# MrOlm/inStrain

Hardware: AMD Instinct MI355X
Metric: Gbp profiled/s (higher is better)
Workload: dtype u32

## Files before the change

include/instrain_amd.h:

```cpp
#ifndef INSTRAIN_AMD_H
#define INSTRAIN_AMD_H

#include <stdint.h>

#ifdef __cplusplus
extern "C" {
#endif

#define ISX_OK 0
#define ISX_ERR_ARG (-1)
#define ISX_ERR_HIP (-2)
#define ISX_ERR_CAPACITY (-3)
#define ISX_ERR_MM_RANGE (-4)
#define ISX_ERR_IO (-5)
#define ISX_ERR_STATE (-6)

#define ISX_ABI_VERSION 5


typedef struct isx_ctx isx_ctx;
typedef struct isx_batch isx_batch;
typedef struct isx_bam isx_bam;
struct isx_bam_params_s;
struct isx_bam_info_s;
// ... 393 lines not shown
    int32_t lev_mask_bytes, lev_cov_bytes, lev_window, n_lev_windows, lev_min_cov, pad_lev;
    uint64_t rows_checksum;
} isx_pipe_result;

int isx_levels_expand(const isx_pipe_result *r, int32_t host_threads, uint32_t *gpos, uint32_t *mm_cov, float *clon, float *clon_rarefied);

int isx_pipe_create(isx_ctx *ctx, const isx_params *params, const isx_pipe_params *pp, isx_pipe **out);
void isx_pipe_destroy(isx_pipe *p);
int isx_pipe_submit(isx_pipe *p, int64_t n_pos, const uint8_t *ref, int32_t n_splits, const int64_t *split_bounds,
                    int64_t n_obs, const isx_obs *obs, const uint32_t *pair, int64_t *ticket);
int isx_pipe_submit_bam(isx_pipe *p, isx_bam *bam, const struct isx_bam_params_s *bp, const int32_t *refs, int32_t n_refs,
                        const uint8_t *ref, int32_t n_splits, const int64_t *split_bounds, struct isx_bam_info_s *info,
                        int64_t *ticket);
int isx_pipe_collect(isx_pipe *p, int64_t ticket, isx_pipe_result *out);
int isx_pipe_release(isx_pipe *p, int64_t ticket);
int isx_pipe_fetch_entries(isx_pipe *p, int64_t ticket, isx_entry *out);
int isx_pipe_fetch_entries_shrunk(isx_pipe *p, int64_t ticket, uint32_t *gpos, uint32_t *mm_cov, float *clon, float *clon_rarefied);


#define ISX_SEG_BASES 150
#define ISX_SEG_WORDS 15
#define ISX_SEG_SKIP_WORD 0x24924924u
#define ISX_DREC_WORDS 8
#define ISX_DREC_EXC 6
#define ISX_DREC_EXC_FULL 3
#define ISX_DREC_DUAL 0x80000000u
#define ISX_DREC_NO_EXC 0x3FFFFFFFu

typedef struct {
    int64_t n_seg;
    const uint32_t *gpos;
    const uint8_t *len;
    const uint8_t *mm;
    const uint32_t *pair;
    const uint32_t *bases;
} isx_segs;

int isx_batch_create_reads(isx_ctx *ctx, const isx_params *params, int64_t n_pos, const uint8_t *ref, int32_t n_splits,
                           const int64_t *split_bounds, const isx_segs *segs, isx_batch **out);
int isx_pipe_submit_reads(isx_pipe *p, int64_t n_pos, const uint8_t *ref, int32_t n_splits, const int64_t *split_bounds,
                          const isx_segs *segs, int64_t *ticket);

typedef struct isx_wire isx_wire;
int isx_pipe_stage_reads(isx_pipe *p, int64_t n_pos, const uint8_t *ref, int32_t n_splits, const int64_t *split_bounds,
                         const isx_segs *segs, isx_wire **out);
int isx_pipe_submit_wire(isx_pipe *p, const isx_wire *wire, int64_t *ticket);
int64_t isx_wire_bytes(const isx_wire *wire);
void isx_wire_free(isx_wire *wire);
int isx_wire_keep_reference(isx_pipe *p, isx_wire *wire);

#define ISX_PLANE_WORDS 8
typedef struct {
    int64_t n_seg;
    const uint32_t *gpos;
    const uint8_t *len;
    const uint32_t *pair;
    const uint64_t *planes;
    const uint8_t *mm;
} isx_read_planes;

typedef struct {
    const uint8_t *plane2;
    const uint8_t *nplane;
    uint64_t key;
} isx_ref_planes;

int isx_pack_ref_planes(const uint8_t *ref, int64_t n_pos, int32_t host_threads, uint8_t *plane2, uint8_t *nplane, int32_t *has_n);
int isx_planes_from_segs(const isx_segs *segs, int32_t host_threads, uint64_t *planes);
int isx_pack_read_planes(int64_t n_reads, const int64_t *ref_start, const int64_t *clip_lo, const int64_t *clip_hi,
                         const uint32_t *cigar, const int64_t *cigar_off, const char *seq, const uint8_t *qual, const int64_t *seq_off,
                         const uint32_t *pair, int32_t min_base_quality, int64_t cap_seg, uint32_t *seg_gpos,
                         uint8_t *seg_len, uint32_t *seg_pair, uint64_t *seg_planes, int64_t *n_seg);
int isx_pipe_submit_planes(isx_pipe *p, int64_t n_pos, const isx_ref_planes *ref, int32_t n_splits, const int64_t *split_bounds,
                           const isx_read_planes *reads, int64_t *ticket);
int isx_pipe_stage_planes(isx_pipe *p, int64_t n_pos, const isx_ref_planes *ref, int32_t n_splits, const int64_t *split_bounds,
                          const isx_read_planes *reads, isx_wire **out);
int isx_pipe_set_reference_budget(isx_pipe *p, int64_t mib);
int isx_host_register(const void *ptr, int64_t bytes);
int isx_host_unregister(const void *ptr);
int isx_encode_planes(const isx_read_planes *reads, const isx_ref_planes *ref, int64_t n_pos, int32_t host_threads, int32_t slack_groups,
                      int64_t cap_rec, int64_t ring_records, uint32_t *rec, uint32_t *gbase, int64_t *n_rec, int64_t *need_slack);
int isx_encode_planes_mm(const isx_read_planes *reads, const isx_ref_planes *ref, int64_t n_pos, int32_t n_mm_bins, int32_t host_threads, int32_t slack_groups,
                         int64_t cap_rec, int64_t ring_records, uint32_t *rec, uint32_t *gbase, int64_t *n_rec, int64_t *need_slack);

int isx_count_read_segs(int64_t n_reads, const uint32_t *cigar, const int64_t *cigar_off, const int64_t *ref_start,
                        const int64_t *clip_lo, const int64_t *clip_hi, int64_t *n_seg);
int isx_pack_reads(int64_t n_reads, const int64_t *ref_start, const int64_t *clip_lo, const int64_t *clip_hi,
                   const uint32_t *cigar, const int64_t *cigar_off, const char *seq, const uint8_t *qual, const int64_t *seq_off,
                   const uint8_t *mm, const uint32_t *pair, int32_t min_base_quality, int64_t cap_seg, uint32_t *seg_gpos,
                   uint8_t *seg_len, uint8_t *seg_mm, uint32_t *seg_pair, uint32_t *seg_bases, int64_t *n_seg);

int isx_encode_segs(const isx_segs *segs, int64_t n_pos, int32_t n_mm_bins, int32_t host_threads, int64_t cap_rec, uint32_t *rec,
                    uint32_t *gbase, uint32_t *pair_out, int64_t *n_rec);
int64_t isx_seg_records_needed(const uint32_t *gpos, int64_t n_seg, int32_t host_threads);
int isx_encode_segs_ring(const isx_segs *segs, int64_t n_pos, int32_t n_mm_bins, int32_t host_threads, int64_t cap_rec, int64_t ring_records,
                         uint32_t *rec, uint32_t *gbase, uint32_t *pair_out, int64_t *n_rec);

int isx_encode_delta(const isx_segs *segs, const uint8_t *ref, int64_t n_pos, int32_t n_mm_bins, int32_t host_threads, int32_t slack_groups,
                     int64_t cap_rec, int64_t ring_records, uint32_t *rec, uint32_t *gbase, uint32_t *pair_out, int64_t *n_rec, int64_t *need_slack);
int64_t isx_delta_records_needed(const uint32_t *gpos, int64_t n_seg, int32_t host_threads, int32_t slack_groups);

int isx_encode_obs(const isx_obs *obs, const uint32_t *pair, int64_t n_obs, int64_t n_pos, int32_t record_bytes,
                   int32_t host_threads, double slack, int64_t cap_rec, void *rec, uint32_t *gbase, uint32_t *pair_out,
                   int64_t *n_rec, int32_t *passes);
int isx_encode_obs_ring(const isx_obs *obs, const uint32_t *pair, int64_t n_obs, int64_t n_pos, int32_t record_bytes,
                        int32_t host_threads, double slack, int64_t cap_rec, int64_t ring_records, void *rec,
                        uint32_t *gbase, uint32_t *pair_out, int64_t *n_rec, int32_t *passes);

typedef struct {
    int64_t in_off;
    int32_t in_len;
    int32_t out_len;
    int64_t out_off;
} isx_bgzf_block;
int isx_bgzf_index(const uint8_t *image, int64_t n_bytes, int64_t cap_blocks, isx_bgzf_block *blocks, int64_t *n_blocks, int64_t *out_bytes);
int isx_bgzf_inflate_device(isx_ctx *ctx, const uint8_t *image, int64_t n_bytes, const isx_bgzf_block *blocks, int64_t n_blocks,
                            uint8_t *out, int64_t out_bytes, float *kernel_ms);
int isx_bgzf_inflate_host(const uint8_t *image, int64_t n_bytes, const isx_bgzf_block *blocks, int64_t n_blocks, uint8_t *out, int64_t out_bytes);
int isx_bgzf_inflate_fast(const uint8_t *image, int64_t n_bytes, const isx_bgzf_block *blocks, int64_t n_blocks, uint8_t *out, int64_t out_bytes);

typedef struct isx_bam_params_s {
    double min_read_ani;
    int32_t min_mapq;
    double max_insert_relative;
    int32_t min_insert;
    int32_t min_base_quality;
    int32_t skip_mm;
    int32_t window_length;
    int32_t pairing_filter;
} isx_bam_params;

typedef struct isx_bam_info_s {
    int32_t n_refs;
    int32_t n_splits;
    int64_t n_reads;
    int64_t n_pos;
    int64_t n_obs;
    int64_t n_pairs;
    int64_t unfiltered_pairs, filtered_pairs;
    int64_t filtered_bases;
    double median_insert;
    int32_t max_mm;
    int32_t pad;
    int64_t unfiltered_reads, unfiltered_singletons, filtered_singletons;
    int64_t n_segs;
} isx_bam_info;

int isx_bam_open(const char *path, isx_bam **out);
void isx_bam_close(isx_bam *bam);
void isx_bam_close_wait(isx_bam *bam);
int isx_bam_set_threads(isx_bam *bam, int32_t threads);
int isx_bam_ref(const isx_bam *bam, int32_t i, const char **name, int64_t *length, int64_t *flat_offset);
int isx_bam_set_priority_reads(isx_bam *bam, int64_t n, const char *names, const int64_t *offs);
int isx_bam_scan(isx_bam *bam, isx_bam_info *info );
int isx_bam_scan_part(isx_bam *bam, int32_t part, int32_t n_parts, isx_bam_info *info );
int isx_bam_set_wanted_refs(isx_bam *bam, const int32_t *refs, int32_t n);
int isx_bam_insert_sizes(isx_bam *bam, int64_t *out, int64_t cap, int64_t *n);
int isx_bam_filter(isx_bam *bam, const isx_bam_params *p, double median_insert , isx_bam_info *info);
int isx_bam_pair_keys(isx_bam *bam, uint64_t *h1, uint64_t *h2, int32_t *tid, int64_t *info4, int64_t cap, int64_t *n);
int isx_bam_set_cross_names(isx_bam *bam, int64_t n, const int64_t *entry, const int64_t *occurrences, const int64_t *info4);
int isx_bam_filter_insert_sizes(isx_bam *bam, int64_t *out, int64_t cap, int64_t *n);
int isx_bam_set_r2m(isx_bam *bam, int32_t ref, int64_t n, const char *names, const int64_t *offs, const int32_t *mm );
int isx_bam_set_mm_cap(isx_bam *bam, int32_t cap);
int isx_bam_mm_levels(const isx_bam *bam, int32_t *levels, int32_t cap, int32_t *n);
int isx_bam_set_mm_levels(isx_bam *bam, const int32_t *levels, int32_t n);
int isx_bam_batch_pair_names(const isx_bam *bam, int64_t *n, int64_t *name_bytes, char *names, int64_t *offs);
// ... 18 lines not shown
```

instrain_amd/_lib.py:

```python
import ctypes as C
import os

import numpy as np

_HERE = os.path.dirname(os.path.abspath(__file__))
LIB_PATH = os.path.join(_HERE, "libinstrain_amd.so")
if os.environ.get("ISX_LIB"):
    LIB_PATH = os.path.abspath(os.environ["ISX_LIB"])

BGZF_BLOCK_DT = np.dtype([("in_off", np.int64), ("in_len", np.int32), ("out_len", np.int32), ("out_off", np.int64)])
OBS_DT = np.dtype([("gpos", "<u4"), ("mm", "<u2"), ("base", "u1"), ("flags", "u1")])
ENTRY_DT = np.dtype([("gpos", "<u4"), ("mm", "<u2"), ("flags", "<u2"), ("cnt", "<u4", (4,)), ("clon", "<f4"),
                     ("clon_rarefied", "<f4")])
SNV_DT = np.dtype([("gpos", "<u4"), ("mm", "<u2"), ("con_base", "u1"), ("var_base", "u1"),
                   ("allele_count", "u1"), ("cls", "u1"), ("cryptic", "u1"), ("ref_base", "u1"),
                   ("cnt", "<u4", (4,))])
LD_DT = np.dtype([("gpos_a", "<u4"), ("gpos_b", "<u4"), ("mm", "<u2"), ("allele_A", "u1"), ("allele_a", "u1"),
                  ("allele_B", "u1"), ("allele_b", "u1"), ("pad", "<u2"), ("total", "<u4"), ("countAB", "<u4"),
                  ("countAb", "<u4"), ("countaB", "<u4"), ("countab", "<u4"), ("pad2", "<u4"),
                  ("r2", "<f8"), ("d_prime", "<f8"), ("r2_normalized", "<f8"), ("d_prime_normalized", "<f8")])
AO_DT = np.dtype([("pair", "<u4"), ("gpos", "<u4"), ("order", "<u4"), ("mm", "<u2"), ("base", "u1"), ("pad", "u1")])
assert AO_DT.itemsize == 16
assert OBS_DT.itemsize == 8 and ENTRY_DT.itemsize == 32 and SNV_DT.itemsize == 28 and LD_DT.itemsize == 72

# ... 73 lines not shown


class BamParams(C.Structure):
    _fields_ = [("min_read_ani", C.c_double), ("min_mapq", C.c_int32), ("max_insert_relative", C.c_double),
                ("min_insert", C.c_int32), ("min_base_quality", C.c_int32), ("skip_mm", C.c_int32),
                ("window_length", C.c_int32), ("pairing_filter", C.c_int32)]


PAIRING_FILTERS = {"paired_only": 0, "non_discordant": 1, "all_reads": 2}


class BamInfo(C.Structure):
    _fields_ = [("n_refs", C.c_int32), ("n_splits", C.c_int32), ("n_reads", C.c_int64), ("n_pos", C.c_int64),
                ("n_obs", C.c_int64), ("n_pairs", C.c_int64), ("unfiltered_pairs", C.c_int64),
                ("filtered_pairs", C.c_int64), ("filtered_bases", C.c_int64), ("median_insert", C.c_double),
                ("max_mm", C.c_int32), ("pad", C.c_int32), ("unfiltered_reads", C.c_int64),
                ("unfiltered_singletons", C.c_int64), ("filtered_singletons", C.c_int64), ("n_segs", C.c_int64)]


SCAFFOLD_LEVEL_DT = np.dtype([("nonzero", "<i8"), ("sum_cov", "<u8"), ("sumsq_cov", "<u8"), ("median_cov", "<f8"),
                              ("counted", "<i8"), ("sum_clon", "<f8"), ("median_clon", "<f8"),
                              ("counted_rarefied", "<i8"), ("sum_clon_rarefied", "<f8"),
                              ("median_clon_rarefied", "<f8"), ("mm", "<i4"), ("present", "<i4")])
assert SCAFFOLD_LEVEL_DT.itemsize == 88
GENOME_LEVEL_DT = np.dtype([("n", "<i8"), ("sum_cov", "<u8"), ("sumsq_cov", "<u8"), ("median_cov", "<f8"), ("mm", "<i4"), ("pad", "<i4")])
assert GENOME_LEVEL_DT.itemsize == 40
GENOME_COV_DT = np.dtype([("n", "<i8"), ("sum_cov", "<u8"), ("sumsq_cov", "<u8"), ("max_cov", "<u4"), ("pad", "<u4")])
SNV_LEVEL_DT = np.dtype([(n, "<u4") for n in ("divergent", "sns", "snv", "con", "pop")])
LD_LEVEL_DT = np.dtype([("n", "<i8"), ("n_r2", "<i8"), ("n_dprime", "<i8"), ("sum_distance", "<i8"), ("sum_r2", "<f8"), ("sum_dprime", "<f8")])
assert GENOME_COV_DT.itemsize == 32 and SNV_LEVEL_DT.itemsize == 20 and LD_LEVEL_DT.itemsize == 48


COMPARE_LEVEL_DT = np.dtype([("both", "<i8"), ("either", "<i8"), ("mm", "<i4"), ("present_a", "<i4"),
                             ("present_b", "<i4"), ("pad", "<i4"), ("consensus_snps", "<i8"), ("population_snps", "<i8")])
assert COMPARE_LEVEL_DT.itemsize == 48
COMPARE_SNP_DT = np.dtype([("gpos", "<u4"), ("mm", "<u2"), ("consensus_snp", "u1"), ("population_snp", "u1"),
                           ("has_a", "u1"), ("has_b", "u1"), ("con_a", "u1"), ("ref_a", "u1"), ("var_a", "u1"),
                           ("con_b", "u1"), ("ref_b", "u1"), ("var_b", "u1"), ("cnt_a", "<u4", (4,)), ("cnt_b", "<u4", (4,))])
assert COMPARE_SNP_DT.itemsize == 48
IREP_WINDOW, IREP_SLIDE = 5000, 100
IREP_GENOME_DT = np.dtype([("L", "<i8"), ("n_blocks", "<i8"), ("n_windows", "<i8"), ("first_block", "<i8"), ("first_window", "<i8"),
                           ("first_scaffold", "<i4"), ("num_contigs", "<i4")])
IREP_ROW_DT = np.dtype([("L", "<i8"), ("n_windows", "<i8"), ("n_kept", "<i8"), ("sum_cov", "<u8"), ("avg_cov", "<f8"), ("fragMbp", "<f8"),
                        ("kept_windows", "<f8"), ("r2", "<f8"), ("raw_irep", "<f8"), ("gc_irep", "<f8"), ("irep", "<f8"),
                        ("num_contigs", "<i4"), ("flags", "<u4")])
assert IREP_GENOME_DT.itemsize == 48 and IREP_ROW_DT.itemsize == 96
IREP_FAIL_KEPT, IREP_FAIL_COV, IREP_FAIL_R2, IREP_FAIL_FRAG, IREP_EMPTY, IREP_NO_FIT = 1, 2, 4, 8, 16, 32
CMPSET_TILE_DT = np.dtype([("word0", "<i8"), ("n_words", "<i4"), ("scaffold", "<i4")])
CMPSET_MAX_LEVELS = 128
POOL_SITE_DT = np.dtype([("gpos", "<u4"), ("n_detect", "<u4"), ("cnt", "<u8", (4,)), ("n_detect_5x", "<u4"), ("cls_count", "<u2", (5,)),
                         ("ref_base", "u1"), ("con_base", "u1"), ("var_base", "u1"), ("n_con_bases", "u1"), ("con_bases", "u1"),
                         ("pad", "u1", (5,))])
assert POOL_SITE_DT.itemsize == 64
POOL_META_HAS, POOL_META_OWN = 1, 2


GENE_DT = np.dtype([("start", "<i8"), ("end", "<i8"), ("seq_off", "<i8"), ("strand", "<i4"), ("pad", "<i4")])
GENE_COV_DT = np.dtype([("sum_cov", "<u8"), ("nonzero", "<u4"), ("counted", "<u4"), ("sum_clon", "<f8")])
GENE_SNV_COUNT_DT = np.dtype([(n, "<u4") for n in ("divergent", "sns", "sns_n", "sns_s", "snv", "snv_n", "snv_s")])
GENE_MUTATION_DT = np.dtype([("gene", "<i4"), ("k", "<i4"), ("type", "u1"), ("aa_old", "u1"), ("aa_new", "u1"), ("n_genes", "u1"),
                             ("pad", "<u4")])
assert GENE_DT.itemsize == 32 and GENE_COV_DT.itemsize == 24 and GENE_SNV_COUNT_DT.itemsize == 28 and GENE_MUTATION_DT.itemsize == 16
GENE_LEVEL_PRESENT, GENE_COV_ANY, GENE_CLON_ANY = 1, 2, 4


ERR_CAPACITY = -3


class IsxError(RuntimeError):
    def __init__(self, code, msg):
        super().__init__("libinstrain_amd error %d: %s" % (code, msg))
        self.code = code


SYMBOLS = ["isx_last_error", "isx_abi_version", "isx_ctx_create", "isx_ctx_destroy", "isx_ctx_reserve_cus", "isx_set_null_model",
           "isx_batch_create", "isx_batch_create_reads", "isx_batch_destroy", "isx_batch_run", "isx_batch_launch", "isx_batch_wait", "isx_batch_sizes", "isx_batch_timings", "isx_batch_link_chain",
           "isx_batch_fetch_entries", "isx_batch_fetch_dense", "isx_batch_fetch_snv", "isx_batch_fetch_ld", "isx_batch_fetch_allele_obs",
           "isx_batch_summarize", "isx_batch_summarize_genomes", "isx_batch_genome_coverage", "isx_snv_level_counts", "isx_ld_level_sums", "isx_compare_coverage", "isx_compare_scaffolds", "isx_compare_fetch_snps",
           "isx_cmpset_layout", "isx_cmpset_tiles", "isx_cmpset_level_map", "isx_cmpset_create", "isx_cmpset_destroy", "isx_cmpset_add", "isx_cmpset_axis", "isx_cmpset_compare", "isx_cmpset_pair_snps", "isx_cmpset_fetch_snps",
           "isx_cmpset_pool_enable", "isx_cmpset_pool_sites", "isx_cmpset_pool_fetch_sites", "isx_cmpset_pool_add", "isx_cmpset_pool_summary", "isx_cmpset_pool_fetch_sample",
           "isx_irep_layout", "isx_irep_create", "isx_irep_destroy", "isx_irep_sizes", "isx_irep_add", "isx_irep_blocks_fetch", "isx_irep_blocks_add", "isx_irep_finish",
           "isx_genes_create", "isx_genes_destroy", "isx_genes_sites", "isx_batch_profile_genes", "isx_genes_profile_snvs",
           "isx_pipe_create", "isx_pipe_destroy", "isx_pipe_submit", "isx_pipe_submit_reads", "isx_pipe_stage_reads", "isx_pipe_submit_wire", "isx_wire_bytes", "isx_wire_free", "isx_wire_keep_reference", "isx_pipe_submit_bam", "isx_encode_segs", "isx_encode_segs_ring", "isx_seg_records_needed", "isx_encode_delta", "isx_delta_records_needed", "isx_count_read_segs", "isx_pack_reads", "isx_pipe_collect", "isx_pipe_release", "isx_pipe_fetch_entries", "isx_pipe_fetch_entries_shrunk", "isx_levels_expand", "isx_encode_obs", "isx_encode_obs_ring",
           "isx_pack_ref_planes", "isx_planes_from_segs", "isx_pack_read_planes", "isx_pipe_submit_planes", "isx_pipe_stage_planes", "isx_encode_planes", "isx_encode_planes_mm", "isx_pipe_set_reference_budget", "isx_host_register", "isx_host_unregister",
           "isx_bgzf_index", "isx_bgzf_inflate_device", "isx_bgzf_inflate_host", "isx_bgzf_inflate_fast",
           "isx_bam_open", "isx_bam_close", "isx_bam_close_wait", "isx_bam_set_threads", "isx_bam_ref", "isx_bam_set_priority_reads", "isx_bam_scan", "isx_bam_scan_part",
           "isx_bam_insert_sizes", "isx_bam_set_wanted_refs", "isx_bam_pair_keys", "isx_bam_set_cross_names", "isx_bam_filter_insert_sizes", "isx_bam_filter", "isx_bam_set_r2m", "isx_bam_r2m", "isx_bam_drop_names", "isx_bam_batch_pair_names", "isx_bam_set_mm_cap", "isx_bam_mm_levels", "isx_bam_set_mm_levels", "isx_bam_ref_counts",
           "isx_bam_expand_refs", "isx_bam_segment_refs", "isx_bam_copy_segs", "isx_bam_copy_read_planes", "isx_bam_expand_region", "isx_bam_expand", "isx_bam_copy", "isx_bam_view"]

_lib = None


def load():
    global _lib
    if _lib is not None:
        return _lib
    if not os.path.exists(LIB_PATH):
        raise IsxError(-2, "%s not built: run `python -c 'import __graft_entry__ as g; g.build()'` "
                           "(hipcc --offload-arch=gfx950)" % LIB_PATH)
    lib = C.CDLL(LIB_PATH)
    vp, i32, i64 = C.c_void_p, C.c_int32, C.c_int64
    lib.isx_last_error.restype = C.c_char_p
    lib.isx_abi_version.restype = C.c_int
    if lib.isx_abi_version() != ABI_VERSION:
        raise IsxError(-6, "%s has ABI version %d, this package binds version %d: rebuild it (python -c 'import __graft_entry__ as g; g.build()')"
                       % (LIB_PATH, lib.isx_abi_version(), ABI_VERSION))
    lib.isx_ctx_create.argtypes = [C.c_int, C.POINTER(vp)]
    lib.isx_ctx_destroy.argtypes = [vp]
    lib.isx_ctx_reserve_cus.argtypes = [vp, C.c_int]
    lib.isx_bgzf_index.argtypes = [vp, i64, i64, vp, C.POINTER(i64), C.POINTER(i64)]
    lib.isx_bgzf_inflate_device.argtypes = [vp, vp, i64, vp, i64, vp, i64, C.POINTER(C.c_float)]
    lib.isx_bgzf_inflate_host.argtypes = [vp, i64, vp, i64, vp, i64]
    lib.isx_bgzf_inflate_fast.argtypes = [vp, i64, vp, i64, vp, i64]
    lib.isx_ctx_destroy.restype = None
    lib.isx_set_null_model.argtypes = [vp, vp, i64, i32]
    lib.isx_batch_create.argtypes = [vp, C.POINTER(Params), i64, vp, i32, vp, i64, vp, vp, C.POINTER(vp)]
    lib.isx_batch_create_reads.argtypes = [vp, C.POINTER(Params), i64, vp, i32, vp, C.POINTER(Segs), C.POINTER(vp)]
    lib.isx_pipe_submit_reads.argtypes = [vp, i64, vp, i32, vp, C.POINTER(Segs), C.POINTER(i64)]
    lib.isx_pipe_stage_reads.argtypes = [vp, i64, vp, i32, vp, C.POINTER(Segs), C.POINTER(vp)]
    lib.isx_pipe_submit_wire.argtypes = [vp, vp, C.POINTER(i64)]
    lib.isx_wire_bytes.argtypes = [vp]
    lib.isx_wire_bytes.restype = i64
    lib.isx_wire_free.argtypes = [vp]
    lib.isx_wire_keep_reference.argtypes = [vp, vp]
    lib.isx_wire_free.restype = None
    lib.isx_encode_segs.argtypes = [C.POINTER(Segs), i64, i32, i32, i64, vp, vp, vp, C.POINTER(i64)]
    lib.isx_encode_segs_ring.argtypes = [C.POINTER(Segs), i64, i32, i32, i64, i64, vp, vp, vp, C.POINTER(i64)]
    lib.isx_encode_delta.argtypes = [C.POINTER(Segs), vp, i64, i32, i32, i32, i64, i64, vp, vp, vp, C.POINTER(i64), C.POINTER(i64)]
    lib.isx_delta_records_needed.argtypes = [vp, i64, i32, i32]
    lib.isx_delta_records_needed.restype = i64
    lib.isx_seg_records_needed.argtypes = [vp, i64, i32]
    lib.isx_seg_records_needed.restype = i64
    lib.isx_count_read_segs.argtypes = [i64, vp, vp, vp, vp, vp, C.POINTER(i64)]
    lib.isx_pack_reads.argtypes = [i64, vp, vp, vp, vp, vp, vp, vp, vp, vp, vp, i32, i64, vp, vp, vp, vp, vp, C.POINTER(i64)]
    lib.isx_batch_destroy.argtypes = [vp]
    lib.isx_batch_destroy.restype = None
    lib.isx_batch_run.argtypes = [vp]
    lib.isx_batch_launch.argtypes = [vp]
    lib.isx_batch_wait.argtypes = [vp]
    lib.isx_batch_sizes.argtypes = [vp, C.POINTER(Sizes)]
    lib.isx_batch_timings.argtypes = [vp, C.POINTER(Timings)]
    lib.isx_batch_link_chain.argtypes = [vp]
    for f in ("isx_batch_fetch_entries", "isx_batch_fetch_snv", "isx_batch_fetch_ld", "isx_batch_fetch_allele_obs"):
        getattr(lib, f).argtypes = [vp, vp]
    lib.isx_batch_fetch_dense.argtypes = [vp, vp, vp, vp]
    lib.isx_batch_summarize.argtypes = [vp, i32, vp, vp, C.POINTER(C.c_float)]
    lib.isx_batch_summarize_genomes.argtypes = [vp, i32, vp, i32, vp, i32, vp, C.POINTER(C.c_float)]
    lib.isx_batch_genome_coverage.argtypes = [vp, i32, vp, vp, i32, i32, i32, vp, vp, C.POINTER(C.c_float)]
    lib.isx_snv_level_counts.argtypes = [vp, i32, vp, i64, vp, i32, vp, C.POINTER(C.c_float)]
    lib.isx_ld_level_sums.argtypes = [vp, i32, vp, i64, vp, i32, vp, C.POINTER(C.c_float)]
    lib.isx_compare_coverage.argtypes = [vp, vp, i32, vp, i32, vp, C.POINTER(C.c_float)]
    lib.isx_compare_scaffolds.argtypes = [vp, vp, i32, vp, i32, C.c_double, vp, C.POINTER(i64), C.POINTER(C.c_float)]
    lib.isx_compare_fetch_snps.argtypes = [vp, vp]
    lib.isx_cmpset_layout.argtypes = [i32, vp, vp]
    lib.isx_cmpset_tiles.argtypes = [i32, vp, i32, vp]
    lib.isx_cmpset_tiles.restype = i64
    lib.isx_cmpset_level_map.argtypes = [i32, vp, vp, i32, vp, C.POINTER(i32), vp]
    lib.isx_cmpset_create.argtypes = [vp, i32, vp, i32, C.POINTER(vp)]
    lib.isx_cmpset_destroy.argtypes = [vp]
    lib.isx_cmpset_destroy.restype = None
    lib.isx_cmpset_add.argtypes = [vp, i32, vp, i32, vp, vp, vp]
    lib.isx_cmpset_axis.argtypes = [vp, C.POINTER(i32), C.POINTER(i32), vp]
    lib.isx_cmpset_compare.argtypes = [vp, C.c_double, i64, vp, C.POINTER(C.c_float)]
    lib.isx_cmpset_pair_snps.argtypes = [vp, i32, i32, C.POINTER(i64)]
    lib.isx_cmpset_fetch_snps.argtypes = [vp, vp]
    lib.isx_cmpset_pool_enable.argtypes = [vp]
    lib.isx_cmpset_pool_sites.argtypes = [vp, C.POINTER(i64)]
    lib.isx_cmpset_pool_fetch_sites.argtypes = [vp, vp]
    lib.isx_cmpset_pool_add.argtypes = [vp, i32, vp, i32, vp, vp]
    lib.isx_cmpset_pool_summary.argtypes = [vp, i64, vp, C.POINTER(C.c_float)]
    lib.isx_cmpset_pool_fetch_sample.argtypes = [vp, i32, vp, vp]
    lib.isx_irep_layout.argtypes = [i32, vp, vp, i32, i32, vp, vp, vp]
    lib.isx_irep_create.argtypes = [vp, i32, vp, vp, i32, i32, C.POINTER(vp)]
    lib.isx_irep_destroy.argtypes = [vp]
    lib.isx_irep_destroy.restype = None
    lib.isx_irep_sizes.argtypes = [vp, C.POINTER(i64), C.POINTER(i32), C.POINTER(i32)]
    lib.isx_irep_add.argtypes = [vp, vp, i32, vp, vp, i32, C.POINTER(C.c_float)]
    lib.isx_irep_blocks_fetch.argtypes = [vp, vp, vp, vp]
    lib.isx_irep_blocks_add.argtypes = [vp, vp, vp, vp]
    lib.isx_irep_finish.argtypes = [vp, vp, C.POINTER(C.c_float)]
    lib.isx_genes_create.argtypes = [vp, i64, vp, C.c_char_p, i64, C.POINTER(vp)]
    lib.isx_genes_destroy.argtypes = [vp]
    lib.isx_genes_destroy.restype = None
    lib.isx_genes_sites.argtypes = [vp, vp, C.POINTER(C.c_float)]
    lib.isx_batch_profile_genes.argtypes = [vp, vp, i32, vp, vp, vp, vp, vp, C.POINTER(C.c_float)]
    lib.isx_genes_profile_snvs.argtypes = [vp, i32, vp, vp, vp, i64, vp, i32, vp, vp, C.POINTER(C.c_float)]
    lib.isx_pipe_create.argtypes = [vp, C.POINTER(Params), C.POINTER(PipeParams), C.POINTER(vp)]
    lib.isx_pipe_destroy.argtypes = [vp]
    lib.isx_pipe_destroy.restype = None
    lib.isx_pipe_submit.argtypes = [vp, i64, vp, i32, vp, i64, vp, vp, C.POINTER(i64)]
    lib.isx_pipe_submit_bam.argtypes = [vp, vp, C.POINTER(BamParams), vp, i32, vp, i32, vp, C.POINTER(BamInfo), C.POINTER(i64)]
    lib.isx_pipe_collect.argtypes = [vp, i64, C.POINTER(PipeResult)]
    lib.isx_pipe_release.argtypes = [vp, i64]
    lib.isx_pipe_fetch_entries.argtypes = [vp, i64, vp]
    lib.isx_pipe_fetch_entries_shrunk.argtypes = [vp, i64, vp, vp, vp, vp]
    lib.isx_levels_expand.argtypes = [C.POINTER(PipeResult), i32, vp, vp, vp, vp]
    lib.isx_encode_obs.argtypes = [vp, vp, i64, i64, i32, i32, C.c_double, i64, vp, vp, vp, C.POINTER(i64), C.POINTER(i32)]
    lib.isx_encode_obs_ring.argtypes = [vp, vp, i64, i64, i32, i32, C.c_double, i64, i64, vp, vp, vp, C.POINTER(i64), C.POINTER(i32)]
    lib.isx_bam_open.argtypes = [C.c_char_p, C.POINTER(vp)]
    lib.isx_bam_close.argtypes = [vp]
    lib.isx_bam_close.restype = None
    lib.isx_bam_close_wait.argtypes = [vp]
    lib.isx_bam_close_wait.restype = None
    lib.isx_bam_expand.argtypes = [vp, C.POINTER(BamParams), C.POINTER(BamInfo)]
    lib.isx_bam_set_threads.argtypes = [vp, i32]
    lib.isx_bam_set_priority_reads.argtypes = [vp, i64, C.c_char_p, vp]
    lib.isx_bam_scan.argtypes = [vp, C.POINTER(BamInfo)]
    lib.isx_bam_scan_part.argtypes = [vp, i32, i32, C.POINTER(BamInfo)]
    lib.isx_bam_set_wanted_refs.argtypes = [vp, vp, i32]
    lib.isx_bam_insert_sizes.argtypes = [vp, vp, i64, C.POINTER(i64)]
    lib.isx_bam_filter_insert_sizes.argtypes = [vp, vp, i64, C.POINTER(i64)]
    lib.isx_bam_pair_keys.argtypes = [vp, vp, vp, vp, vp, i64, C.POINTER(i64)]
    lib.isx_bam_set_cross_names.argtypes = [vp, i64, vp, vp, vp]
    lib.isx_bam_filter.argtypes = [vp, C.POINTER(BamParams), C.c_double, C.POINTER(BamInfo)]
    lib.isx_bam_set_r2m.argtypes = [vp, i32, i64, C.c_char_p, vp, vp]
    lib.isx_bam_drop_names.argtypes = [vp]
    lib.isx_bam_r2m.argtypes = [vp, i32, C.POINTER(i64), C.POINTER(i64), vp, vp, vp]
    lib.isx_bam_batch_pair_names.argtypes = [vp, C.POINTER(i64), C.POINTER(i64), vp, vp]
    lib.isx_bam_set_mm_cap.argtypes = [vp, i32]
    lib.isx_bam_mm_levels.argtypes = [vp, vp, i32, vp]
    lib.isx_bam_set_mm_levels.argtypes = [vp, vp, i32]
    lib.isx_bam_ref_counts.argtypes = [vp, vp, vp]
    lib.isx_bam_expand_region.argtypes = [vp, C.POINTER(BamParams), i32, i64, i64, C.POINTER(BamInfo)]
    lib.isx_bam_expand_refs.argtypes = [vp, C.POINTER(BamParams), vp, i32, C.POINTER(BamInfo)]
    lib.isx_bam_segment_refs.argtypes = [vp, C.POINTER(BamParams), vp, i32, C.POINTER(BamInfo), C.POINTER(i64)]
    lib.isx_bam_copy_segs.argtypes = [vp, vp, vp, vp, vp, vp, vp, vp]
    lib.isx_bam_copy_read_planes.argtypes = [vp, vp]
    lib.isx_pack_ref_planes.argtypes = [vp, i64, i32, vp, vp, C.POINTER(i32)]
    lib.isx_planes_from_segs.argtypes = [C.POINTER(Segs), i32, vp]
    lib.isx_pack_read_planes.argtypes = [i64, vp, vp, vp, vp, vp, vp, vp, vp, vp, i32, i64, vp, vp, vp, vp, C.POINTER(i64)]
    lib.isx_pipe_submit_planes.argtypes = [vp, i64, C.POINTER(RefPlanes), i32, vp, C.POINTER(ReadPlanes), C.POINTER(i64)]
    lib.isx_pipe_set_reference_budget.argtypes = [vp, i64]
    lib.isx_host_register.argtypes = [vp, i64]
    lib.isx_host_unregister.argtypes = [vp]
    lib.isx_pipe_stage_planes.argtypes = [vp, i64, C.POINTER(RefPlanes), i32, vp, C.POINTER(ReadPlanes), C.POINTER(vp)]
    lib.isx_encode_planes.argtypes = [C.POINTER(ReadPlanes), C.POINTER(RefPlanes), i64, i32, i32, i64, i64, vp, vp, C.POINTER(i64), C.POINTER(i64)]
    lib.isx_encode_planes_mm.argtypes = [C.POINTER(ReadPlanes), C.POINTER(RefPlanes), i64, i32, i32, i32, i64, i64, vp, vp, C.POINTER(i64), C.POINTER(i64)]
    lib.isx_bam_ref.argtypes = [vp, i32, C.POINTER(C.c_char_p), C.POINTER(i64), C.POINTER(i64)]
    lib.isx_bam_copy.argtypes = [vp, vp, vp, vp, vp]
    lib.isx_bam_view.argtypes = [vp, C.POINTER(vp), C.POINTER(vp)]
    _lib = lib
    return lib


def check(rc):
    if rc != 0:
        raise IsxError(rc, load().isx_last_error().decode(errors="replace"))
```

instrain_amd/csrc/isx_api.hip:

```cpp
#include <algorithm>
#include <atomic>
#include <cmath>
#include <chrono>
#include <cstdlib>
#include <cstring>
#include <map>
#include <mutex>
#include <string>
#include <unordered_map>
#include <thread>
#include <type_traits>
#include <vector>
#include <unistd.h>
#include <sys/prctl.h>
#include <time.h>

#include "isx_batch.h"
#include "seg_encode.h"

static thread_local std::string g_err;
void isx_set_error(const std::string &msg) { g_err = msg; }

namespace {
struct BlockCache {
// ... 661 lines not shown
            launch_extract_gpos(b->d_rec, b->d_rec32, b->d_gbase, b->d_gpos, b->d_gpos16, b->d_rec32 ? b->d_gbase : b->d_cbase,
                                b->d_rec32 ? ISX_GROUP : ISX_CHUNK, b->n_rec, c->stream);
            HIP_TRY(isx_wait_stream(c->stream));
        }
        uint32_t maxp = 0;
        const int rc = staged_upload(c, b->d_pair, b->n_rec, [&](uint32_t *dst, uint64_t first, uint64_t cnt) {
            if (og_start.empty()) {
                for (uint64_t i = 0; i < cnt; i++) {
                    const uint64_t g = first + i;
                    dst[i] = g < (uint64_t)n_obs ? pair[g] : 0u;
                    if (g < (uint64_t)n_obs) maxp = std::max(maxp, pair[g]);
                }
            } else {
                for (uint64_t i0 = 0; i0 < cnt; i0 += G) {
                    const uint64_t dg = (first + i0) / G;
                    const uint64_t n_real = dg < og_start.size() ? og_count[dg] : 0;
                    for (uint64_t i = 0; i < n_real; i++) { dst[i0 + i] = pair[og_start[dg] + i]; maxp = std::max(maxp, dst[i0 + i]); }
                    for (uint64_t i = n_real; i < G; i++) dst[i0 + i] = 0u;
                }
            }
        });
        b->n_pairs = (uint64_t)maxp + 1;
        return rc;
    }
};


void batch_pick_block(isx_batch *b)
{
    if (b->M == 1) { b->block = 1024; return; }
    b->block = 512;
    if (b->prm.window > 0) { if (b->prm.window > 1024) b->block = 1024; return; }
    if (batch_window_for(b, b->n_pos, true) < 1024) b->block = 1024;
}

int batch_window_for(const isx_batch *b, int64_t n_pos, bool packed)
{
    const isx_params *prm = &b->prm;
    if (prm->window > 0) return prm->window;
    if (b->M == 1) {
        const int64_t wsmall = (n_pos / 1024 + 63) / 64 * 64;
        if (wsmall < 2048) return (int)std::max<int64_t>(512, wsmall);
        int best = 2560;
        double best_eff = 0.0;
        const int wtop = (b->drec && packed) ? (prm->enable_linkage ? 4352 : 6080)
                       : b->drec ? (prm->enable_linkage ? 2688 : 3264)
                                 : (prm->enable_linkage ? 3136 : ISX_PK16_MAX_W);
        for (int w = 2048; w <= wtop; w += 64) {
            const double n_win = std::ceil((double)n_pos / w);
            const double rounds = n_win / (2.0 * b->ctx->pass_cus);
            const double eff = rounds / std::ceil(rounds) * (w / (w + 200.0));
            if (eff > best_eff + 1e-9) { best_eff = eff; best = w; }
        }
        return best;
    }
    const int bytes_per_pos = b->M * ((packed ? 8 : 16) + (b->drec ? (packed ? 4 : 8) : 0)) + ((b->M + 31) / 32) * 4 + 5;
    const int budget = (b->block >= 1024 ? 156 : 78) * 1024;
    const int wmax = ((budget - 8 * b->qcap - 8192 - 2048 - 256) / bytes_per_pos) / 64 * 64;
    return std::min(std::max(wmax, 64), 2 * b->block);
}

static uint64_t build_window_directory(const uint32_t *cmin, const uint32_t *cmax, const uint8_t *cany, uint64_t n_chunks, int W,
                                       int64_t n_pos, std::vector<uint2> &win, uint32_t chunk)
{
    std::vector<uint32_t> pmax(n_chunks), smin(n_chunks);
    uint32_t run = 0;
    for (uint64_t i = 0; i < n_chunks; i++) { if (cany[i]) run = std::max(run, cmax[i]); pmax[i] = run; }
    run = 0xFFFFFFFFu;
    for (uint64_t i = n_chunks; i-- > 0;) { if (cany[i]) run = std::min(run, cmin[i]); smin[i] = run; }
    const int n_win = (int)((n_pos + W - 1) / W);
    win.assign((size_t)n_win, make_uint2(0, 0));
    uint64_t lo = 0, hi = 0, longest = 0;
    for (int w = 0; w < n_win; w++) {
        const uint64_t w0 = (uint64_t)w * W, w1 = w0 + W;
        while (lo < n_chunks && (uint64_t)pmax[lo] < w0) lo++;
        if (hi < lo) hi = lo;
        while (hi < n_chunks && (uint64_t)smin[hi] < w1) hi++;
        win[(size_t)w] = make_uint2((uint32_t)(lo * chunk), (uint32_t)(hi * chunk));
        longest = std::max(longest, (hi - lo) * chunk);
    }
    return longest;
}

static uint64_t build_window_directory_mt(isxenc::HostPool &pool, const uint32_t *cmin, const uint32_t *cmax, const uint8_t *cany, uint64_t n_chunks, int W,
                                          int64_t n_pos, std::vector<uint2> &win, uint32_t chunk, std::vector<uint32_t> &pmax, std::vector<uint32_t> &smin)
{
    const int n_win = (int)((n_pos + W - 1) / W);
    const int T = std::min(pool.size(), 16);
    if (T < 2 || n_chunks < 4096 || n_win < 1024) return build_window_directory(cmin, cmax, cany, n_chunks, W, n_pos, win, chunk);
    if (pmax.size() < n_chunks) { pmax.resize(n_chunks); smin.resize(n_chunks); }
    const uint64_t B = (n_chunks + (uint64_t)T - 1) / (uint64_t)T;
    uint32_t bmax[16], bmin[16], cmax_in[16], cmin_in[16];
    pool.run(T, [&](int t) {
        const uint64_t a = std::min(n_chunks, B * (uint64_t)t), e = std::min(n_chunks, a + B);
        uint32_t run = 0;
        for (uint64_t i = a; i < e; i++) { if (cany[i]) run = std::max(run, cmax[i]); pmax[i] = run; }
        bmax[t] = run;
        run = 0xFFFFFFFFu;
        for (uint64_t i = e; i-- > a;) { if (cany[i]) run = std::min(run, cmin[i]); smin[i] = run; }
        bmin[t] = run;
    });
    { uint32_t run = 0; for (int t = 0; t < T; t++) { cmax_in[t] = run; run = std::max(run, bmax[t]); } }
    { uint32_t run = 0xFFFFFFFFu; for (int t = T; t-- > 0;) { cmin_in[t] = run; run = std::min(run, bmin[t]); } }
    auto PM = [&](uint64_t i) { return std::max(pmax[i], cmax_in[i / B]); };
    auto SM = [&](uint64_t i) { return std::min(smin[i], cmin_in[i / B]); };
    win.resize((size_t)n_win);
    uint64_t longest_t[16];
    pool.run(T, [&](int t) {
        const int wa = (int)((int64_t)n_win * t / T), we = (int)((int64_t)n_win * (t + 1) / T);
        uint64_t longest = 0, lo = 0, hi = 0;
        if (wa < we) {
            const uint64_t w0 = (uint64_t)wa * (uint64_t)W;
            uint64_t l = 0, r = n_chunks;
            while (l < r) { const uint64_t m = (l + r) >> 1; if ((uint64_t)PM(m) < w0) l = m + 1; else r = m; }
            lo = hi = l;
        }
        for (int w = wa; w < we; w++) {
            const uint64_t w0 = (uint64_t)w * (uint64_t)W, w1 = w0 + (uint64_t)W;
            while (lo < n_chunks && (uint64_t)PM(lo) < w0) lo++;
            if (hi < lo) hi = lo;
            while (hi < n_chunks && (uint64_t)SM(hi) < w1) hi++;
            win[(size_t)w] = make_uint2((uint32_t)(lo * chunk), (uint32_t)(hi * chunk));
            longest = std::max(longest, (hi - lo) * chunk);
        }
        longest_t[t] = longest;
    });
    uint64_t longest = 0;
    for (int t = 0; t < T; t++) longest = std::max(longest, longest_t[t]);
    if (getenv("ISX_DIR_CHECK")) {
        std::vector<uint2> ref;
        const uint64_t l2 = build_window_directory(cmin, cmax, cany, n_chunks, W, n_pos, ref, chunk);
        if (l2 != longest || ref.size() != win.size() || memcmp(ref.data(), win.data(), ref.size() * sizeof(uint2)) != 0) {
            fprintf(stderr, "build_window_directory_mt differs from build_window_directory (%llu chunks, %d windows)\n", (unsigned long long)n_chunks, n_win);
            abort();
        }
    }
    return longest;
}

int choose_windows(const isx_batch *b, int64_t n_pos, const ChunkDir &dir, DirThreads *mt, std::vector<uint2> &win, int *packed)
{
    auto build = [&](int W) {
        return mt ? build_window_directory_mt(mt->pool, dir.cmin, dir.cmax, dir.cany, dir.n_chunks, W, n_pos, win, dir.chunk, mt->pmax, mt->smin)
                  : build_window_directory(dir.cmin, dir.cmax, dir.cany, dir.n_chunks, W, n_pos, win, dir.chunk);
    };
    *packed = 0;
    if ((b->M > 1 || b->drec) && !(b->prm.layout & ISX_LAYOUT_NO_PACKED_COUNTERS)) {
        const int Wp = batch_window_for(b, n_pos, true);
        if (build(Wp) < (b->drec ? 32768u : 65536u)) { *packed = 1; return Wp; }
    }
    const int W = batch_window_for(b, n_pos, false);
    build(W);
    return W;
}

int check_split_bounds(int64_t n_pos, int32_t n_splits, const int64_t *split_bounds)
{
    if (split_bounds[0] != 0 || split_bounds[n_splits] != n_pos) { isx_set_error("split_bounds must span [0, n_pos]"); return ISX_ERR_ARG; }
    for (int i = 0; i < n_splits; i++)
        if (split_bounds[i + 1] <= split_bounds[i]) { isx_set_error("split_bounds must be strictly ascending"); return ISX_ERR_ARG; }
    return ISX_OK;
}

int seg_status_error(int erc, const char *capacity_text, int capacity_code)
{
    switch (erc) {
    case isxenc::SEG_OK: return ISX_OK;
    case isxenc::SEG_CAPACITY: isx_set_error(capacity_text); return capacity_code;
    case isxenc::SEG_MM_RANGE: isx_set_error("a segment has mm >= n_mm_bins"); return ISX_ERR_MM_RANGE;
    case isxenc::SEG_BAD_POS: isx_set_error("a segment reaches beyond n_pos"); return ISX_ERR_ARG;
    default: isx_set_error("a segment's length is not in [1, 150]"); return ISX_ERR_ARG;
    }
}

int batch_set_geometry(isx_batch *b)
{
    const bool dense = b->M == 1;
    if (!dense && b->W > 2 * b->block) { isx_set_error("mm path: window must be <= 2 x block"); return ISX_ERR_ARG; }
    if (b->drec && dense && b->W > (b->packed ? 8 : 4) * b->block) { isx_set_error("reference-delta records: window must be <= 4 x block (8 x with 16-bit counters)"); return ISX_ERR_ARG; }
    b->rqcap = dense ? 0 : std::min(b->W, 512);
    b->lds = pileup_lds_bytes(b->W, b->M, b->qcap, b->rqcap, b->prm.enable_linkage, b->packed, b->block, b->segs ? (b->drec ? 32 : 64) : 0, &b->stage_off, &b->dlt_off);
    if (b->lds > 160 * 1024) { isx_set_error("window * n_mm_bins does not fit the 160 KiB LDS"); return ISX_ERR_ARG; }
    {
        const int per_cu = std::max(1, std::min((int)(160 * 1024 / b->lds), 2048 / b->block));
        int g = b->ctx->pass_cus * per_cu;
#ifdef ISX_TUNING
        if (const char *e = getenv("ISX_GRID")) g = std::max(8, atoi(e));
#endif
        g = std::min(g, b->n_win);
        b->grid = std::max(8, (g + 7) / 8 * 8);
    }
    if (!dense) {
        b->slab = (uint32_t)b->W * (uint32_t)std::min(b->M, 4);
        if (!b->cap_ovf) {
            const uint64_t npm = (uint64_t)b->n_pos * b->M;
            b->cap_ovf = b->M <= 4 ? 16 : (size_t)std::max<uint64_t>(1u << 20, std::min<uint64_t>((uint64_t)b->n_obs, npm) / 4);
        }
    }
    return ISX_OK;
}


extern "C" {

const char *isx_last_error(void) { return g_err.c_str(); }
int isx_abi_version(void) { return ISX_ABI_VERSION; }

static int make_pass_queues(isx_ctx *c, int r, int n_cu)
{
    r = std::max(0, std::min(r, 8));
    if (n_cu != 256) r = 0;
    for (int i = 0; i < 2; i++) if (c->pstream[i]) { HIP_TRY(isx_wait_stream(c->pstream[i])); HIP_TRY(hipStreamDestroy(c->pstream[i])); c->pstream[i] = nullptr; }
    for (int k = 0; k < 8; k++) c->side_mask[k] = 0;
    c->pass_cus = 256;
    if (r > 0) {
        uint32_t mask[8];
        for (int k = 0; k < 8; k++) {
            mask[k] = 0xFFFFFFFFu;
            for (int j = 0; j < r; j++) mask[k] &= ~(1u << (((k + (j >> 2)) & 7) + 8 * (j & 3)));
        }
        bool ok = true;
        for (int i = 0; i < 2 && ok; i++) ok = hipExtStreamCreateWithCUMask(&c->pstream[i], 8, mask) == hipSuccess;
        if (ok) {
            c->pass_cus = 256 - 8 * r;
            if (!getenv("ISX_SIDE_UNMASKED")) for (int k = 0; k < 8; k++) c->side_mask[k] = ~mask[k];
        } else {
            (void)hipGetLastError();
            for (int i = 0; i < 2; i++) if (c->pstream[i]) { (void)hipStreamDestroy(c->pstream[i]); c->pstream[i] = nullptr; }
            r = 0;
        }
// ... 974 lines not shown
```

instrain_amd/csrc/isx_batch.h:

```cpp
#pragma once
#include <vector>

#include "isx_internal.h"
#include "isx_linkage.h"
#include "isx_summary.h"

namespace isxenc { class HostPool; }

struct isx_ctx {
    int device = 0;
    hipStream_t stream = nullptr;
    hipStream_t pstream[2] = {nullptr, nullptr};
    uint32_t side_mask[8] = {0, 0, 0, 0, 0, 0, 0, 0};
    int pass_cus = 256;
    struct isx_batch *unpublished[2] = {nullptr, nullptr};
    unsigned n_created = 0;
    unsigned n_pipes = 0;
    uint8_t *d_lut = nullptr;
    std::vector<int32_t> h_lut;
    int32_t lut_n = 0, fallback = 0;
    void *pin[2] = {nullptr, nullptr};
    hipEvent_t pin_ev[2] = {nullptr, nullptr};
    size_t pin_bytes = 0;
};
// ... 32 lines not shown
    uint2 *d_win = nullptr;
    uint16_t *d_thr = nullptr;
    int qcap = 1024, rqcap = 0, stage_off = 0;
    bool in_flight = false, publish_enqueued = true, tim_pending = false;
    int ps = 0;
    int64_t *d_bounds = nullptr;
    uint4 *d_counts = nullptr;
    float *d_clon = nullptr;
    float *d_clon_r = nullptr;
    uint16_t *d_cov16 = nullptr;
    uint2 *d_rare = nullptr;
    size_t cap_rare = 0;
    uint32_t n_rare = 0, n_sat = 0;
    uint8_t *d_cov8 = nullptr;
    uint2 *d_sat = nullptr, *d_clon_list = nullptr, *d_clon_sorted = nullptr;
    size_t cap_sat = 0, cap_clon = 0;
    uint32_t n_clon = 0;
    int spin_us = 2000;
    bool nib_pass = false;
    bool nib_out = false;
    uint32_t *d_cov_row_win = nullptr;
    size_t cap_cov_row_win = 0;
    uint32_t n_cov_rows = 0;
    bool sparse_out = false, cov8_out = false;
    bool rare_dense = true;
    bool lean = false, clon_dense = false;
    bool lev_sparse = false;
    void *d_lev_mask = nullptr, *d_lev_cov = nullptr;
    uint32_t *d_lev_win_off = nullptr;
    size_t cap_lev = 0;
    int lev_mask_bytes = 0, lev_cov_bytes = 1;
    isx_entry *d_entries = nullptr;
    uint32_t *d_win_nent = nullptr;
    uint32_t *d_win_site_base = nullptr, *d_win_site_cnt = nullptr;
    size_t cap_win_sites = 0;
    bool sites_loose = false;
    isx_slev *d_slev = nullptr;
    uint32_t slab = 0;
    size_t cap_ovf = 0, cap_slev = 0;
    isx_snv *d_snv = nullptr;
    isx_site *d_sites = nullptr;
    isx_snv *d_snv_raw = nullptr;
    isx_site *d_sites_raw = nullptr;
    uint2 *d_rare_raw = nullptr;
    uint32_t *d_win_rec = nullptr, *d_win_out = nullptr;
    size_t cap_snv_raw = 0, cap_sites_raw = 0, cap_rare_raw = 0, cap_win = 0;
    bool ordered = false;
    isx_ao *d_ao = nullptr;
    uint32_t *d_cursors = nullptr, *d_flags = nullptr;
    uint32_t *h_state = nullptr;
    uint32_t *d_host_state = nullptr;
    uint32_t base[CUR_N] = {};
    uint32_t epoch = 0;
    size_t cap_entries = 0, cap_snv = 0, cap_sites = 0, cap_ao = 0;
    LinkageBuffers L;
    const isx_ld *ld_host = nullptr;
    size_t n_ld_host = 0;
    uint32_t n_ao_pass = 0;
    int link_chain = 0;
    SummaryBuffers S;
    CompareBuffers C;
    hipEvent_t ev_sum[2] = {};
    hipEvent_t ev[10] = {};
    bool ran = false;
    uint32_t n_ovf = 0;
    isx_sizes sizes{};
    isx_timings tim{};
};


static inline uint32_t entry_wins(const isx_batch *b) { return b->lev_sparse ? 0u : (uint32_t)b->n_win; }

std::vector<uint16_t> build_thresholds(const std::vector<int32_t> &lut, int32_t fallback, double min_freq);

void batch_pick_block(isx_batch *b);
int batch_window_for(const isx_batch *b, int64_t n_pos, bool packed);

int check_split_bounds(int64_t n_pos, int32_t n_splits, const int64_t *split_bounds);

int seg_status_error(int erc, const char *capacity_text, int capacity_code);

struct ChunkDir { const uint32_t *cmin, *cmax; const uint8_t *cany; uint64_t n_chunks; uint32_t chunk; };
struct DirThreads { isxenc::HostPool &pool; std::vector<uint32_t> &pmax, &smin; };
int choose_windows(const isx_batch *b, int64_t n_pos, const ChunkDir &dir, DirThreads *mt, std::vector<uint2> &win, int *packed);

int batch_set_geometry(isx_batch *b);

extern "C" {
int launch_pass(isx_batch *b);
int finish_pass(isx_batch *b, uint32_t *cap_flags, hipStream_t link_stream = nullptr);
int finish_pass_sizes(isx_batch *b, uint32_t *cap_flags, hipStream_t link_stream = nullptr);
int finish_pass_link(isx_batch *b, hipStream_t link_stream = nullptr);
int batch_grow_tables(isx_batch *b, uint32_t cap_flags);
void fill_summary_in(isx_batch *b, int32_t n_scaffolds, const int64_t *scaffold_bounds, SummaryIn &in);
}
```

instrain_amd/csrc/isx_pipe.hip:

```cpp
#include <atomic>
#include <algorithm>
#include <chrono>
#include <cmath>
#include <condition_variable>
#include <cstring>
#include <deque>
#include <mutex>
#include <memory>
#include <string>
#include <thread>
#include <vector>

#include "bam_front.h"
#include "isx_batch.h"
#include "obs_encode.h"
#include "seg_encode.h"
#include "isx_summary.h"
#include <unordered_map>

namespace {

constexpr size_t ALIGN = 256;
inline size_t up(size_t v, size_t a = ALIGN) { return (v + a - 1) / a * a; }

double now_ms()
{
    return std::chrono::duration<double, std::milli>(std::chrono::steady_clock::now().time_since_epoch()).count();
}

int host_block_alloc(void **p, size_t bytes, bool pinned)
{
    *p = nullptr;
    if (pinned) { HIP_TRY(isx_pin_malloc(p, std::max<size_t>(bytes, 1))); return ISX_OK; }
    if (posix_memalign(p, 4096, std::max<size_t>(bytes, 4096)) != 0) { *p = nullptr; isx_set_error("out of host memory"); return ISX_ERR_ARG; }
    return ISX_OK;
}

void host_block_free(void *p, bool pinned)
{
    if (!p) return;
    if (pinned) isx_pin_free(p); else free(p);
}

static const bool pipe_timing = getenv("ISX_PIPE_TIMING") != nullptr;
#define H2D(p, s) ((s).h2d ? (s).h2d : (p)->s_h2d)
struct Slot {
    isx_batch *b = nullptr;
    hipStream_t h2d = nullptr;
    uint8_t *h_in = nullptr, *d_in = nullptr;
    size_t in_bytes = 0;
    size_t off_bounds = 0, off_win = 0, off_ref = 0, off_gbase = 0, off_ridx = 0, off_rec = 0;
    size_t off_pairs = 0;
    isxenc::PairRun *h_runs = nullptr;
    bool runs_pinned = true;
    uint2 *d_runs = nullptr;
    size_t cap_runs = 0;
    hipEvent_t ev_ring[2] = {nullptr, nullptr};
    bool ring_busy[2] = {false, false};
    uint8_t *h_out = nullptr;
    uint8_t *h_small = nullptr;
    size_t small_bytes = 0;
    bool out_pinned = true;
    size_t out_bytes = 0, o_counts = 0, o_clon = 0, o_clonr = 0, o_snv = 0, o_cov16 = 0, o_rare = 0;
    bool rare_dense = false;
    bool cov8 = false, clon_sparse = false;
    bool cov4 = false;
    size_t cov_rows_off = 0;
    int cov_window = 0;
    std::vector<uint32_t> cov_row_win;
    std::vector<isx_sat> sat_rows;
    bool sat_complete = true;
    void *sort_temp = nullptr;
    size_t sort_temp_bytes = 0;
    std::vector<float> clonr_big;
    std::vector<isx_rare> rare_big;
    std::vector<uint32_t> cmin, cmax, dir_pmax, dir_smin;
    std::vector<uint8_t> cany;
    std::vector<uint2> win;
    size_t o_lmask = 0, o_lwin = 0, o_lcov = 0, o_lclon = 0, o_lrare = 0;
    size_t lcov_room = 0, lclon_room = 0, lrare_room = 0;
    std::vector<uint8_t> lcov_big;
    std::vector<isx_rare> lclon_big, lrare_big;
    std::vector<isx_snv> snv_big;
    std::vector<isx_ld> ld_rows;
    uint64_t rows_checksum = 0;
    hipEvent_t ev_h2d0 = nullptr, ev_h2d1 = nullptr, ev_pass = nullptr, ev_d2h0 = nullptr, ev_d2h1 = nullptr;
    hipEvent_t ev_h2da = nullptr, ev_h2db = nullptr;
    bool h2d_split = false;
    int64_t ticket = -1;
    BamBatch *dead_batch = nullptr;
    bool ref_has_n = false;
    int state = 0;
    int rc = 0;
    std::string err;
    float finish_wait_ms = 0.f;
    float encode_ms = 0.f;
    int encode_passes = 0;
    int64_t h2d_bytes = 0, d2h_bytes = 0;
    uint16_t *d_gpos16 = nullptr;
};

static uint64_t bytes_checksum(const void *p, size_t bytes, uint64_t seed)
{
    const uint8_t *b = static_cast<const uint8_t *>(p);
    uint64_t a[4] = {seed ^ 0x9E3779B97F4A7C15ull, seed + 0xC2B2AE3D27D4EB4Full, seed ^ 0x165667B19E3779F9ull, seed + 0x27D4EB2F165667C5ull};
    const size_t n8 = bytes / 8;
    size_t i = 0;
    for (; i + 4 <= n8; i += 4) {
        uint64_t w[4];
        memcpy(w, b + 8 * i, 32);
        for (int k = 0; k < 4; k++) a[k] = a[k] * 0x100000001B3ull + w[k];
    }
    uint64_t h = (uint64_t)bytes;
    for (; i < n8; i++) { uint64_t w; memcpy(&w, b + 8 * i, 8); h = h * 0x100000001B3ull + w; }
    for (size_t j = n8 * 8; j < bytes; j++) h = h * 0x100000001B3ull + b[j];
    for (int k = 0; k < 4; k++) { h ^= a[k]; h *= 0xFF51AFD7ED558CCDull; h ^= h >> 33; }
    return h;
}

static inline size_t ref2_bytes(int64_t n_pos) { return (((size_t)n_pos + 3) / 4 + 15) & ~(size_t)15; }
static inline size_t refn_bytes(int64_t n_pos) { return (((size_t)n_pos + 7) / 8 + 15) & ~(size_t)15; }

static bool copy_ref_planes(isxenc::HostPool &pool, const isx_ref_planes *rp, int64_t n_pos, uint8_t *plane2, uint8_t *nplane)
{
    const size_t b2 = ((size_t)n_pos + 3) / 4, bn = ((size_t)n_pos + 7) / 8;
    const size_t piece = (size_t)1 << 20;
    const int t2 = (int)((b2 + piece - 1) / piece), tn = rp->nplane ? (int)((bn + piece - 1) / piece) : 0;
    std::atomic<int> any{0};
    pool.run(t2 + tn, [&](int t) {
        if (t < t2) { const size_t a = (size_t)t * piece; memcpy(plane2 + a, rp->plane2 + a, std::min(piece, b2 - a)); return; }
        const size_t a = (size_t)(t - t2) * piece, n = std::min(piece, bn - a);
        const uint8_t *src = rp->nplane + a;
        uint8_t acc = 0;
        for (size_t i = 0; i < n; i++) acc |= src[i];
        memcpy(nplane + a, src, n);
// ... 801 lines not shown
                s.d2h_bytes += (int64_t)n_pos * 4;
            }
        }
    }
    HIP_TRY(hipEventRecord(s.ev_d2h1, p->s_d2h));
    launch_lk.unlock();
    {
        std::lock_guard<std::mutex> lk(p->mu);
        s.ticket = p->next_ticket++;
        if (p->next_promise < p->next_ticket) p->next_promise = p->next_ticket;
        s.state = 1; s.rc = ISX_OK;
        *ticket = s.ticket;
        p->work.push_back(s.ticket);
    }
    p->cv_work.notify_one();
    return ISX_OK;
}


static int check_capacity(const isx_pipe *p, const char *who, int64_t n_pos, int64_t n_items, int64_t max_items, int32_t n_splits)
{
    if (n_pos > p->pp.max_pos || n_items > max_items || n_splits > p->pp.max_splits) {
        isx_set_error(std::string(who) + ": batch larger than the pipe was created for");
        return ISX_ERR_CAPACITY;
    }
    return ISX_OK;
}

static int slot_acquire(isx_pipe *p, const char *who, Slot **out)
{
    Slot &s = p->slots[(size_t)(p->next_ticket % (int64_t)p->slots.size())];
    {
        std::lock_guard<std::mutex> lk(p->mu);
        if (s.state != 0) { isx_set_error(std::string(who) + ": every slot is in use (collect + release the oldest batch first)"); return ISX_ERR_STATE; }
    }
    HIP_TRY(hipSetDevice(p->ctx->device));
    *out = &s;
    return ISX_OK;
}

static int queue_for_stager(isx_pipe *p, isx_pipe::StageJob &&job, const char *who, int64_t *ticket)
{
    const int rc = check_capacity(p, who, job.n_pos, job.planes ? job.reads.n_seg : job.segs.n_seg, p->pp.max_segs, (int32_t)job.bounds.size() - 1);
    if (rc != ISX_OK) return rc;
    {
        std::lock_guard<std::mutex> lk(p->mu);
        const int64_t t = p->next_promise, n = (int64_t)p->slots.size();
        const Slot &s = p->slots[(size_t)(t % n)];
        if (t - n >= p->next_ticket || s.state != 0) { isx_set_error(std::string(who) + ": every slot is in use (collect + release the oldest batch first)"); return ISX_ERR_STATE; }
        job.ticket = t;
        p->next_promise = t + 1;
        *ticket = t;
        p->stage_q.push_back(std::move(job));
    }
    p->cv_stage.notify_one();
    return ISX_OK;
}

struct RingFeed { hipError_t err = hipSuccess; size_t bytes = 0; };

static int ring_feed_install(isx_pipe *p, Slot &s, RingFeed &r, int64_t &ring_groups, std::function<void(int)> &wave_begin,
                             std::function<void(int, int64_t, int64_t)> &wave_flush)
{
    if (p->ring_half <= 0) return ISX_OK;
    HIP_TRY(hipEventRecord(s.ev_h2d0, H2D(p, s)));
    const size_t half_bytes = (size_t)p->ring_half * (size_t)p->rb, grp_bytes = (size_t)p->G * (size_t)p->rb;
    uint8_t *d_rec = s.d_in + s.off_rec;
    ring_groups = p->ring_half / (int64_t)p->G;
    wave_begin = [&s, &r](int h) {
        if (s.ring_busy[h]) { const hipError_t e = isx_wait_event(s.ev_ring[h]); if (e != hipSuccess && r.err == hipSuccess) r.err = e; s.ring_busy[h] = false; }
    };
    wave_flush = [p, &s, &r, half_bytes, grp_bytes, d_rec](int h, int64_t g0, int64_t g1) {
        const size_t n = (size_t)(g1 - g0) * grp_bytes;
        if (g0 == 0) r.bytes = 0;
        hipError_t e = hipMemcpyAsync(d_rec + (size_t)g0 * grp_bytes, s.h_in + s.off_rec + (size_t)h * half_bytes, n, hipMemcpyHostToDevice, H2D(p, s));
        if (e == hipSuccess) e = hipEventRecord(s.ev_ring[h], H2D(p, s));
        if (e != hipSuccess && r.err == hipSuccess) r.err = e;
        s.ring_busy[h] = true;
        r.bytes += n;
    };
    return ISX_OK;
}

static int slot_choose_windows(isx_pipe *p, Slot &s, uint32_t chunk, bool threads)
{
    isx_batch *b = s.b;
    DirThreads mt{*p->pool, s.dir_pmax, s.dir_smin};
    const ChunkDir dir{s.cmin.data(), s.cmax.data(), s.cany.data(), b->n_rec / chunk, chunk};
    b->W = choose_windows(b, b->n_pos, dir, threads ? &mt : nullptr, s.win, &b->packed);
    b->n_win = (int)s.win.size();
    if (s.win.size() > (size_t)p->pp.max_pos / 64 + 2) { isx_set_error("internal: window directory larger than the arena"); return ISX_ERR_STATE; }
    memcpy(s.h_in + s.off_win, s.win.data(), s.win.size() * sizeof(uint2));
    return ISX_OK;
}

constexpr double COV8_BELOW_DEPTH = 16.0;
constexpr double NIB_BELOW_DEPTH = 6.0;
constexpr double LEV_COV8_BELOW_DEPTH = 64.0;
constexpr double RARE_DENSE_OBS_FACTOR = 4.0;

static int slot_shape_pass(isx_pipe *p, Slot &s)
{
    isx_batch *b = s.b;
    const bool dense = b->M == 1;
    const double n_obs = (double)b->n_obs, n_pos = (double)b->n_pos;
    b->sparse_out = dense && b->d_clon_list != nullptr;
    b->cov8_out = b->sparse_out && n_obs < COV8_BELOW_DEPTH * n_pos;
    b->nib_out = b->cov8_out && b->lean && n_obs < NIB_BELOW_DEPTH * n_pos;
    b->clon_dense = false;
    b->rare_dense = !(b->lean && b->sparse_out) || n_obs * RARE_DENSE_OBS_FACTOR >= (double)p->prm.rarefied_coverage * n_pos;
    if (b->lev_sparse) b->lev_cov_bytes = n_obs < LEV_COV8_BELOW_DEPTH * n_pos ? 1 : 2;
    const int rc = batch_set_geometry(b);
    if (rc != ISX_OK) return rc;
    if (!dense && !b->lev_sparse) {
        const size_t used = (size_t)b->n_win * b->slab;
        if (used > b->slab_region) { isx_set_error("internal: entry slabs larger than the slot's region"); return ISX_ERR_STATE; }
        b->cap_ovf = b->cap_entries - used;
    }
    return ISX_OK;
}

static void slot_bind_inputs(isx_pipe *p, Slot &s, uint8_t *resident_ref)
{
    isx_batch *b = s.b;
    const bool linkage = p->prm.enable_linkage != 0;
    uint8_t *rec = s.d_in + s.off_rec;
    b->d_bounds = reinterpret_cast<int64_t *>(s.d_in + s.off_bounds);
    b->d_win = reinterpret_cast<uint2 *>(s.d_in + s.off_win);
    b->d_ref = resident_ref ? resident_ref : s.d_in + s.off_ref;
    b->d_ref_n = s.ref_has_n ? b->d_ref + ref2_bytes(b->n_pos) : nullptr;
    b->d_gbase = reinterpret_cast<uint32_t *>(s.d_in + s.off_gbase);
    b->d_rec16 = p->rb == 2 ? reinterpret_cast<uint16_t *>(rec) : nullptr;
    b->d_rec32 = p->rb == 4 ? reinterpret_cast<uint32_t *>(rec) : nullptr;
    if (p->segs) {
        b->d_seg = p->drec ? nullptr : reinterpret_cast<uint4 *>(rec);
        b->d_drec = p->drec ? reinterpret_cast<uint4 *>(rec) : nullptr;
        b->d_pair = linkage && !p->drec ? reinterpret_cast<uint32_t *>(s.d_in + s.off_pairs) : nullptr;
        b->d_pair_runs = nullptr; b->d_run_index = nullptr; b->n_runs = 0;
    } else {
        b->d_pair = nullptr;
        b->d_pair_runs = linkage ? s.d_runs : nullptr;
        b->d_run_index = linkage ? reinterpret_cast<uint32_t *>(s.d_in + s.off_ridx) : nullptr;
        b->d_gpos16 = s.d_gpos16; b->gpos16_shift = 5;
    }
}

static void ref_cache_insert(isx_pipe *p, Slot &s, const isx_ref_planes *rp, int64_t n_pos)
{
    const size_t rb_all = ref2_bytes(n_pos) + (s.ref_has_n ? refn_bytes(n_pos) : 0);
    if (p->ref_cache_bytes + rb_all > p->ref_cache_budget.load(std::memory_order_relaxed)) return;
    isx_pipe::RefEntry e;
    bool ok = isx_dev_malloc(reinterpret_cast<void **>(&e.d), rb_all + 64) == hipSuccess && hipEventCreateWithFlags(&e.ready, hipEventDisableTiming) == hipSuccess;
    ok = ok && hipMemcpyAsync(e.d, s.d_in + s.off_ref, rb_all, hipMemcpyDeviceToDevice, H2D(p, s)) == hipSuccess && hipEventRecord(e.ready, H2D(p, s)) == hipSuccess;
    if (ok) {
        e.bytes = rb_all; e.n_pos = n_pos; e.has_n = s.ref_has_n; e.sum = ref_plane_checksum(rp->plane2, n_pos);
        p->ref_cache_bytes += rb_all;
        p->ref_cache.emplace(rp->key, e);
    } else {
        if (e.d) isx_dev_free(e.d);
        if (e.ready) (void)hipEventDestroy(e.ready);
        (void)hipGetLastError();
    }
}

struct RefStage {
    bool early = false;
    uint8_t *resident = nullptr;
    double host_ms = 0.0;
};

static int stage_reference(isx_pipe *p, Slot &s, int64_t n_pos, const uint8_t *ref, const isx_ref_planes *rp, isxenc::SegJob &J, RefStage *out)
{
// ... 114 lines not shown
                t_enc - t0, J.passes, now_ms() - t_enc, (long long)n_obs, (long long)J.n_runs);

    if (!ring) HIP_TRY(hipEventRecord(s.ev_h2d0, H2D(p, s)));
    const size_t ref_bytes = ref2_bytes(n_pos) + (s.ref_has_n ? refn_bytes(n_pos) : 0);
    const size_t head = (size_t)(n_splits + 1) * sizeof(int64_t) + s.win.size() * sizeof(uint2) + ref_bytes;
    memset(s.h_in + s.off_gbase + (size_t)(b->n_rec / p->G) * sizeof(uint32_t), 0, ISX_TAIL_GROUPS * sizeof(uint32_t));
    const size_t gb_bytes = ((size_t)(b->n_rec / p->G) + ISX_TAIL_GROUPS) * sizeof(uint32_t), rec_bytes = (size_t)b->n_rec * p->rb + ISX_TAIL_BYTES;
    HIP_TRY(hipMemcpyAsync(s.d_in + s.off_bounds, s.h_in + s.off_bounds, (size_t)(n_splits + 1) * sizeof(int64_t), hipMemcpyHostToDevice, H2D(p, s)));
    HIP_TRY(hipMemcpyAsync(s.d_in + s.off_win, s.h_in + s.off_win, s.win.size() * sizeof(uint2), hipMemcpyHostToDevice, H2D(p, s)));
    HIP_TRY(hipMemcpyAsync(s.d_in + s.off_ref, s.h_in + s.off_ref, ref_bytes, hipMemcpyHostToDevice, H2D(p, s)));
    HIP_TRY(hipMemcpyAsync(s.d_in + s.off_gbase, s.h_in + s.off_gbase, gb_bytes, hipMemcpyHostToDevice, H2D(p, s)));
    if (ring) {
        if (p->rb == 2) HIP_TRY(hipMemsetD8Async(reinterpret_cast<hipDeviceptr_t>(d_rec + (size_t)b->n_rec * 2), 0xFF, ISX_TAIL_BYTES, H2D(p, s)));
        else HIP_TRY(hipMemsetD32Async(reinterpret_cast<hipDeviceptr_t>(d_rec + (size_t)b->n_rec * 4), (int)ISX_PAD32, ISX_TAIL_BYTES / 4, H2D(p, s)));
        if (feed.bytes != (size_t)b->n_rec * p->rb) { isx_set_error("internal: the staging ring did not carry the whole stream"); return ISX_ERR_STATE; }
    } else {
        if (p->rb == 2) memset(s.h_in + s.off_rec + (size_t)b->n_rec * 2, 0xFF, ISX_TAIL_BYTES);
        else std::fill_n(reinterpret_cast<uint32_t *>(s.h_in + s.off_rec + (size_t)b->n_rec * 4), ISX_TAIL_BYTES / 4, (uint32_t)ISX_PAD32);
        HIP_TRY(hipMemcpyAsync(d_rec, s.h_in + s.off_rec, rec_bytes, hipMemcpyHostToDevice, H2D(p, s)));
    }
    s.h2d_bytes = (int64_t)(head + gb_bytes + rec_bytes);
    if (linkage) {
        const size_t rb = (size_t)b->n_runs * sizeof(isxenc::PairRun), ib = (size_t)(b->n_rec / ISX_CHUNK) * sizeof(uint32_t);
        HIP_TRY(hipMemcpyAsync(s.d_runs, s.h_runs, rb, hipMemcpyHostToDevice, H2D(p, s)));
        HIP_TRY(hipMemcpyAsync(s.d_in + s.off_ridx, s.h_in + s.off_ridx, ib, hipMemcpyHostToDevice, H2D(p, s)));
        s.h2d_bytes += (int64_t)(rb + ib);
    }
    HIP_TRY(hipEventRecord(s.ev_h2d1, H2D(p, s)));
    s.h2d_split = false;

    return enqueue_pass(p, s, n_pos, ticket);
}

static int encode_reads(isx_pipe *p, Slot &s, isxenc::SegJob &J, bool planes_in, RingFeed &feed)
{
    s.encode_passes = 1;
    if (!p->drec) return isxenc::encode_segs(*p->pool, J);
    std::vector<int64_t> exact;
    for (int attempt = 0;; attempt++) {
        J.slack_groups = p->dslack;
        J.task_groups = exact.empty() ? nullptr : exact.data();
        feed.bytes = 0;
        const int erc = planes_in ? isxenc::encode_planes(*p->pool, J) : isxenc::encode_delta(*p->pool, J);
        if (erc != isxenc::SEG_CAPACITY || J.need_slack <= p->dslack || attempt != 0) return erc;
        exact = J.task_need;
        int64_t tot = 0;
        for (int64_t v : exact) tot += v;
        const int64_t n_t = (int64_t)exact.size(), base_tot = J.n_rec / ISX_DREC_GROUP - n_t * p->dslack;
        p->dslack = std::max<int64_t>(p->dslack, 1 + (tot - base_tot + n_t - 1) / std::max<int64_t>(n_t, 1));
        s.encode_passes = 2;
    }
}

static int submit_segs_common(isx_pipe *p, int64_t n_pos, const uint8_t *ref, int32_t n_splits, const int64_t *split_bounds,
                              isxenc::SegJob &J, int64_t *ticket, const isx_ref_planes *rp)
{
    static const char who[] = "isx_pipe_submit_reads";
    const bool planes_in = J.in2.planes != nullptr || (bool)J.produce_planes || (J.n_seg == 0 && rp != nullptr);
    int rc;
    if ((rc = check_capacity(p, who, n_pos, J.n_seg, p->pp.max_segs, n_splits)) != ISX_OK) return rc;
    if ((rc = check_split_bounds(n_pos, n_splits, split_bounds)) != ISX_OK) return rc;
    Slot *slot = nullptr;
    if ((rc = slot_acquire(p, who, &slot)) != ISX_OK) return rc;
    Slot &s = *slot;
    isx_batch *b = s.b;
    const bool linkage = p->prm.enable_linkage != 0;

    const double t0 = now_ms();
    J.n_pos = n_pos; J.n_mm_bins = b->M;
    J.rec = reinterpret_cast<uint32_t *>(s.h_in + s.off_rec);
    J.gbase = reinterpret_cast<uint32_t *>(s.h_in + s.off_gbase);
    J.pair_out = linkage && !p->drec ? reinterpret_cast<uint32_t *>(s.h_in + s.off_pairs) : nullptr;
    J.cmin = s.cmin.data(); J.cmax = s.cmax.data(); J.cany = s.cany.data();
    J.cap_rec = p->cap_rec;
    const bool ring = p->ring_half > 0;
    RingFeed feed;
    if ((rc = ring_feed_install(p, s, feed, J.ring_groups, J.wave_begin, J.wave_flush)) != ISX_OK) return rc;
    RefStage rs;
    if (planes_in) {
        if (!p->drec) { isx_set_error("bit-plane reads need a pipe whose batches travel as reference-delta records (one mm bin, or ISX_LAYOUT_MM_DELTA_RECORDS)"); return ISX_ERR_STATE; }
        if ((rc = stage_reference(p, s, n_pos, ref, rp, J, &rs)) != ISX_OK) return rc;
    }
    if (p->drec) J.ref = ref;
    const int erc = encode_reads(p, s, J, planes_in, feed);
    const double t_enc = now_ms();
    if (feed.err != hipSuccess) { isx_set_error(std::string("isx_pipe_submit_reads: staging ring: ") + hipGetErrorString(feed.err)); return ISX_ERR_HIP; }
    if ((rc = seg_status_error(erc, "isx_pipe_submit_reads: the stream jumps too often for the pipe's record capacity (raise jump_slack)", ISX_ERR_CAPACITY)) != ISX_OK) return rc;
    if (J.n_bases > p->pp.max_obs) { isx_set_error("isx_pipe_submit_reads: more bases than the pipe's max_obs"); return ISX_ERR_CAPACITY; }
    bool early_rec = false;
    if (rs.early && !ring) {
        const size_t gb_bytes0 = (size_t)(J.n_rec / (int64_t)p->G) * sizeof(uint32_t), rec_bytes0 = (size_t)J.n_rec * (size_t)p->rb;
        HIP_TRY(hipEventRecord(s.ev_h2db, H2D(p, s)));
        if (s.off_pairs == s.off_rec && s.off_ridx == s.off_rec && s.off_rec - s.off_gbase < ((size_t)2 << 20)) {
            HIP_TRY(hipMemcpyAsync(s.d_in + s.off_gbase, s.h_in + s.off_gbase, (s.off_rec - s.off_gbase) + rec_bytes0, hipMemcpyHostToDevice, H2D(p, s)));
        } else {
            HIP_TRY(hipMemcpyAsync(s.d_in + s.off_gbase, s.h_in + s.off_gbase, gb_bytes0, hipMemcpyHostToDevice, H2D(p, s)));
            HIP_TRY(hipMemcpyAsync(s.d_in + s.off_rec, s.h_in + s.off_rec, rec_bytes0, hipMemcpyHostToDevice, H2D(p, s)));
        }
        early_rec = true;
    }
    if (!planes_in) s.ref_has_n = isxenc::pack_ref_planes(*p->pool, ref, n_pos, s.h_in + s.off_ref, s.h_in + s.off_ref + ref2_bytes(n_pos));
    const double t_ref = now_ms();
    memcpy(s.h_in + s.off_bounds, split_bounds, (size_t)(n_splits + 1) * sizeof(int64_t));

    b->n_pos = n_pos; b->n_obs = J.n_bases; b->n_splits = n_splits; b->n_rec = (uint64_t)J.n_rec;
    b->n_pairs = (uint64_t)J.max_pair + 1;
    if ((rc = slot_choose_windows(p, s, p->G, true)) != ISX_OK) return rc;
    if ((rc = slot_shape_pass(p, s)) != ISX_OK) return rc;
    slot_bind_inputs(p, s, rs.resident);
    s.encode_ms = (float)(now_ms() - t0);
    if (pipe_timing)
        fprintf(stderr, "[isx_pipe_submit_reads] records %.2f ms, reference %.2f ms, bounds + windows %.2f ms; %lld segments, %lld records%s\n",
                t_enc - t0 - rs.host_ms, t_ref - t_enc + rs.host_ms, now_ms() - t_ref, (long long)J.n_seg, (long long)J.n_rec, planes_in ? " (bit planes)" : "");
    const double t_q0 = now_ms();

    if (!ring && !rs.early) HIP_TRY(hipEventRecord(s.ev_h2d0, H2D(p, s)));
    const size_t ref_bytes = ref2_bytes(n_pos) + (s.ref_has_n ? refn_bytes(n_pos) : 0);
    const size_t head = (size_t)(n_splits + 1) * sizeof(int64_t) + s.win.size() * sizeof(uint2) + ref_bytes;
    const size_t gb_bytes = (size_t)(b->n_rec / p->G) * sizeof(uint32_t), rec_bytes = (size_t)b->n_rec * (size_t)p->rb;
    if (s.off_win - s.off_bounds < ((size_t)1 << 20)) {
        HIP_TRY(hipMemcpyAsync(s.d_in + s.off_bounds, s.h_in + s.off_bounds, (s.off_win - s.off_bounds) + s.win.size() * sizeof(uint2), hipMemcpyHostToDevice, H2D(p, s)));
    } else {
        HIP_TRY(hipMemcpyAsync(s.d_in + s.off_bounds, s.h_in + s.off_bounds, (size_t)(n_splits + 1) * sizeof(int64_t), hipMemcpyHostToDevice, H2D(p, s)));
        HIP_TRY(hipMemcpyAsync(s.d_in + s.off_win, s.h_in + s.off_win, s.win.size() * sizeof(uint2), hipMemcpyHostToDevice, H2D(p, s)));
    }
    if (!rs.early) HIP_TRY(hipMemcpyAsync(s.d_in + s.off_ref, s.h_in + s.off_ref, ref_bytes, hipMemcpyHostToDevice, H2D(p, s)));
    if (!early_rec) HIP_TRY(hipMemcpyAsync(s.d_in + s.off_gbase, s.h_in + s.off_gbase, gb_bytes, hipMemcpyHostToDevice, H2D(p, s)));
    if (ring) { if (feed.bytes != rec_bytes) { isx_set_error("internal: the staging ring did not carry the whole stream"); return ISX_ERR_STATE; } }
    else if (!early_rec) HIP_TRY(hipMemcpyAsync(s.d_in + s.off_rec, s.h_in + s.off_rec, rec_bytes, hipMemcpyHostToDevice, H2D(p, s)));
    s.h2d_bytes = (int64_t)(head + gb_bytes + rec_bytes) - (rs.resident ? (int64_t)ref_bytes : 0);
    if (linkage && !p->drec) {
        HIP_TRY(hipMemcpyAsync(s.d_in + s.off_pairs, s.h_in + s.off_pairs, (size_t)b->n_rec * sizeof(uint32_t), hipMemcpyHostToDevice, H2D(p, s)));
        s.h2d_bytes += (int64_t)b->n_rec * 4;
    }
    HIP_TRY(hipEventRecord(s.ev_h2d1, H2D(p, s)));
    s.h2d_split = early_rec;
    const double t_q1 = now_ms();
    rc = enqueue_pass(p, s, n_pos, ticket);
    if (pipe_timing) fprintf(stderr, "[isx_pipe_submit_reads] copy-in queue %.2f ms, pass + copy-out queue %.2f ms\n", t_q1 - t_q0, now_ms() - t_q1);
    return rc;
}

struct isx_wire {
    isx_pipe *pipe = nullptr;
    uint8_t *h = nullptr;
    size_t bytes = 0;
    size_t o_bounds = 0, o_win = 0, o_ref = 0, o_gbase = 0, o_pairs = 0, o_rec = 0;
    size_t bounds_bytes = 0, win_bytes = 0, ref_bytes = 0, gbase_bytes = 0, pairs_bytes = 0, rec_bytes = 0;
    int64_t n_pos = 0, n_bases = 0, n_rec = 0, n_seg = 0;
    int32_t n_splits = 0;
    uint64_t n_pairs = 0;
    int W = 0, packed = 0;
    bool ref_has_n = false;
    float stage_ms = 0.f;
    int encode_passes = 1;
    uint8_t *d_ref = nullptr;
    int device = 0;
};

static int stage_common(isx_pipe *p, int64_t n_pos, const uint8_t *ref, const isx_ref_planes *rp, int32_t n_splits, const int64_t *split_bounds,
                        const isx_segs *segs, const isx_read_planes *reads, isx_wire **out)
{
    isx_segs as_segs{};
    if (reads) { as_segs.n_seg = reads->n_seg; as_segs.gpos = reads->gpos; as_segs.len = reads->len; as_segs.pair = reads->pair; segs = &as_segs; }
    *out = nullptr;
    if (!p->segs) { isx_set_error("isx_pipe_stage_reads: not a read-level pipe (isx_pipe_params.max_segs == 0)"); return ISX_ERR_STATE; }
    const bool linkage = p->prm.enable_linkage != 0;
    if (linkage && segs->n_seg && !segs->pair) { isx_set_error("linkage needs the pair array"); return ISX_ERR_ARG; }
    int rc;
    if ((rc = check_capacity(p, "isx_pipe_stage_reads", n_pos, segs->n_seg, p->pp.max_segs, n_splits)) != ISX_OK) return rc;
    if ((rc = check_split_bounds(n_pos, n_splits, split_bounds)) != ISX_OK) return rc;
    HIP_TRY(hipSetDevice(p->ctx->device));
    const double t0 = now_ms();
    std::unique_ptr<isx_wire, void (*)(isx_wire *)> w(new isx_wire(), isx_wire_free);
    w->pipe = p; w->n_pos = n_pos; w->n_splits = n_splits; w->n_seg = segs->n_seg;
    const isx_batch *b0 = p->slots[0].b;
    const int M = b0->M;
    const size_t G = p->G, rb = (size_t)p->rb;
    auto up = [](size_t v) { return (v + 255) & ~(size_t)255; };
    isxenc::SegJob J;
    std::vector<uint32_t> cmin, cmax;
    std::vector<uint8_t> cany;
    std::vector<int64_t> exact;
    for (int attempt = 0;; attempt++) {
        int64_t cap = p->drec ? isxenc::delta_groups_needed(*p->pool, segs->gpos, segs->n_seg, p->dslack) * ISX_DREC_GROUP
                              : isxenc::seg_groups_needed(*p->pool, segs->gpos, segs->n_seg) * ISX_SEG_GROUP;
        if (!exact.empty()) { cap = 0; for (int64_t v : exact) cap += std::max<int64_t>(v, 1) * ISX_DREC_GROUP; }
        if (cap > p->cap_rec) { isx_set_error("isx_pipe_stage_reads: the stream needs more records than the pipe's capacity (raise jump_slack)"); return ISX_ERR_CAPACITY; }
        const size_t n_groups = (size_t)cap / G;
        w->bounds_bytes = (size_t)(n_splits + 1) * sizeof(int64_t);
// ... 459 lines not shown
```

instrain_amd/csrc/obs_encode.cpp:

```cpp
#include "obs_encode.h"

#include <immintrin.h>
#include <sched.h>

#include <algorithm>
#include <atomic>
#include <cstdio>
#include <cstring>
#include <map>
#include <string>

namespace isxenc {

namespace {

constexpr uint32_t G16 = 512, G32 = 256, CHUNK = 1024, PADREC = 2048;
constexpr uint32_t PAD32 = 0x0700FFFFu;

bool have_avx512()
{
    static const bool v = __builtin_cpu_supports("avx512f") && __builtin_cpu_supports("avx512bw") && __builtin_cpu_supports("avx512vl");
    return v;
}

std::vector<int> parse_cpulist(const std::string &s)
{
    std::vector<int> out;
    size_t i = 0;
    while (i < s.size()) {
        char *end = nullptr;
        const long a = strtol(s.c_str() + i, &end, 10);
        if (end == s.c_str() + i) break;
        long b = a;
        i = (size_t)(end - s.c_str());
        if (i < s.size() && s[i] == '-') { b = strtol(s.c_str() + i + 1, &end, 10); i = (size_t)(end - s.c_str()); }
        for (long c = a; c <= b; c++) out.push_back((int)c);
        while (i < s.size() && (s[i] == ',' || s[i] == '\n' || s[i] == ' ')) i++;
    }
    return out;
}

std::string slurp(const std::string &path)
{
    std::string out;
    if (FILE *f = fopen(path.c_str(), "r")) {
        char buf[4096];
        size_t n;
        while ((n = fread(buf, 1, sizeof buf, f)) > 0) out.append(buf, n);
        fclose(f);
    }
    return out;
}

std::vector<std::vector<int>> l3_domains(int numa_node)
{
    cpu_set_t allowed;
    CPU_ZERO(&allowed);
    if (sched_getaffinity(0, sizeof allowed, &allowed) != 0) return {};
    std::vector<int> cpus;
    if (numa_node >= 0) cpus = parse_cpulist(slurp("/sys/devices/system/node/node" + std::to_string(numa_node) + "/cpulist"));
    if (cpus.empty()) for (int c = 0; c < CPU_SETSIZE; c++) if (CPU_ISSET(c, &allowed)) cpus.push_back(c);
    std::map<std::string, std::vector<int>> by_l3;
    for (int c : cpus) {
        if (!CPU_ISSET(c, &allowed)) continue;
        std::string key = slurp("/sys/devices/system/cpu/cpu" + std::to_string(c) + "/cache/index3/shared_cpu_list");
        if (key.empty()) key = "all";
        by_l3[key].push_back(c);
    }
    std::vector<std::vector<int>> out;
    for (auto &kv : by_l3) out.push_back(kv.second);
    return out;
}

}

HostPool::HostPool(int n_threads, int numa_node, bool pin)
{
    n_threads = std::max(1, n_threads);
    std::vector<std::vector<int>> dom;
    if (pin) dom = l3_domains(numa_node);
    cpus_.resize((size_t)n_threads);
    if (!dom.empty())
        for (int i = 0; i < n_threads; i++) cpus_[(size_t)i] = dom[(size_t)i % dom.size()];
    for (int i = 1; i < n_threads; i++) th_.emplace_back(&HostPool::worker, this, i);
}

HostPool::~HostPool()
{
    {
        std::lock_guard<std::mutex> lk(mu_);
        stop_ = true;
    }
    cv_.notify_all();
    for (auto &t : th_) t.join();
}

void HostPool::worker(int idx)
{
    if (!cpus_[(size_t)idx].empty()) {
        cpu_set_t s;
        CPU_ZERO(&s);
        for (int c : cpus_[(size_t)idx]) CPU_SET(c, &s);
        (void)sched_setaffinity(0, sizeof s, &s);
    }
    uint64_t seen = 0;
    std::unique_lock<std::mutex> lk(mu_);
    for (;;) {
        cv_.wait(lk, [&] { return stop_ || gen_ != seen; });
        if (stop_) return;
        seen = gen_;
        while (next_ < n_tasks_) {
            const int t = next_++;
            const auto *fn = fn_;
            lk.unlock();
            (*fn)(t);
            lk.lock();
        }
        if (--running_ == 0) cv_done_.notify_all();
    }
}

void HostPool::run(int n_tasks, const std::function<void(int)> &fn)
{
    if (n_tasks <= 0) return;
    std::unique_lock<std::mutex> lk(mu_);
    fn_ = &fn; n_tasks_ = n_tasks; next_ = 0;
    running_ = (int)th_.size() + 1;
    ++gen_;
    lk.unlock();
    cv_.notify_all();
    lk.lock();
    while (next_ < n_tasks_) {
        const int t = next_++;
        lk.unlock();
        fn(t);
        lk.lock();
    }
    --running_;
    cv_done_.wait(lk, [&] { return running_ == 0; });
    fn_ = nullptr;
}

namespace {

void stat_scalar(const isx_obs *s, size_t n, uint32_t &lo, uint32_t &hi, uint32_t &mm)
{
    uint32_t l = 0xFFFFFFFFu, h = 0, m = 0;
    for (size_t i = 0; i < n; i++) {
        const uint32_t g = s[i].gpos;
        l = g < l ? g : l; h = g > h ? g : h; m = s[i].mm > m ? s[i].mm : m;
    }
    lo = l; hi = h; mm = m;
}

__attribute__((target("avx512f,avx512bw,avx512vl")))
void stat_avx512(const isx_obs *s, size_t n, uint32_t &lo, uint32_t &hi, uint32_t &mm)
{
    __m512i vlo = _mm512_set1_epi32(-1), vhi = _mm512_setzero_si512(), vmm = _mm512_setzero_si512();
    const __m512i m16 = _mm512_set1_epi32(0xFFFF);
    size_t i = 0;
    for (; i + 8 <= n; i += 8) {
        const __m512i v = _mm512_loadu_si512(reinterpret_cast<const void *>(s + i));
        vlo = _mm512_mask_min_epu32(vlo, 0x5555, vlo, v);
        vhi = _mm512_mask_max_epu32(vhi, 0x5555, vhi, v);
        vmm = _mm512_mask_max_epu32(vmm, 0xAAAA, vmm, _mm512_and_si512(v, m16));
    }
    uint32_t l = _mm512_mask_reduce_min_epu32(0x5555, vlo), h = _mm512_mask_reduce_max_epu32(0x5555, vhi);
    uint32_t m = _mm512_mask_reduce_max_epu32(0xAAAA, vmm);
    for (; i < n; i++) {
        const uint32_t g = s[i].gpos;
        l = g < l ? g : l; h = g > h ? g : h; m = s[i].mm > m ? s[i].mm : m;
    }
    lo = l; hi = h; mm = m;
}

void enc16_scalar(const isx_obs *s, size_t n, uint32_t lo, uint16_t *d)
{
    for (size_t i = 0; i < n; i++) {
        const uint32_t bc = s[i].base > 4 ? 4u : (uint32_t)s[i].base;
        d[i] = (uint16_t)((s[i].gpos - lo) | (bc << 13));
    }
}

void enc32_scalar(const isx_obs *s, size_t n, uint32_t lo, uint32_t *d)
{
    for (size_t i = 0; i < n; i++) {
        const uint32_t bc = s[i].base > 4 ? 4u : (uint32_t)s[i].base;
        d[i] = (s[i].gpos - lo) | ((uint32_t)s[i].mm << 16) | (bc << 24);
    }
}

__attribute__((target("avx512f,avx512bw,avx512vl")))
void enc16_avx512(const isx_obs *s, size_t n, uint32_t lo, uint16_t *d)
{
    const __m512i ie = _mm512_setr_epi32(0, 2, 4, 6, 8, 10, 12, 14, 16, 18, 20, 22, 24, 26, 28, 30);
    const __m512i io = _mm512_setr_epi32(1, 3, 5, 7, 9, 11, 13, 15, 17, 19, 21, 23, 25, 27, 29, 31);
    const __m512i vlo = _mm512_set1_epi32((int)lo), four = _mm512_set1_epi32(4), m8 = _mm512_set1_epi32(0xFF);
    const bool aligned = (reinterpret_cast<uintptr_t>(d) & 31u) == 0;
    size_t i = 0;
    for (; i + 16 <= n; i += 16) {
        const __m512i a = _mm512_loadu_si512(reinterpret_cast<const void *>(s + i));
        const __m512i b = _mm512_loadu_si512(reinterpret_cast<const void *>(s + i + 8));
        const __m512i g = _mm512_permutex2var_epi32(a, ie, b), o = _mm512_permutex2var_epi32(a, io, b);
        const __m512i bs = _mm512_min_epu32(_mm512_and_si512(_mm512_srli_epi32(o, 16), m8), four);
        const __m512i r = _mm512_or_si512(_mm512_sub_epi32(g, vlo), _mm512_slli_epi32(bs, 13));
        const __m256i out = _mm512_cvtepi32_epi16(r);
        if (aligned) _mm256_stream_si256(reinterpret_cast<__m256i *>(d + i), out);
        else _mm256_storeu_si256(reinterpret_cast<__m256i *>(d + i), out);
    }
    enc16_scalar(s + i, n - i, lo, d + i);
}

__attribute__((target("avx512f,avx512bw,avx512vl")))
void enc32_avx512(const isx_obs *s, size_t n, uint32_t lo, uint32_t *d)
{
    const __m512i ie = _mm512_setr_epi32(0, 2, 4, 6, 8, 10, 12, 14, 16, 18, 20, 22, 24, 26, 28, 30);
    const __m512i io = _mm512_setr_epi32(1, 3, 5, 7, 9, 11, 13, 15, 17, 19, 21, 23, 25, 27, 29, 31);
    const __m512i vlo = _mm512_set1_epi32((int)lo), four = _mm512_set1_epi32(4), m8 = _mm512_set1_epi32(0xFF);
    const bool aligned = (reinterpret_cast<uintptr_t>(d) & 63u) == 0;
    size_t i = 0;
    for (; i + 16 <= n; i += 16) {
        const __m512i a = _mm512_loadu_si512(reinterpret_cast<const void *>(s + i));
        const __m512i b = _mm512_loadu_si512(reinterpret_cast<const void *>(s + i + 8));
// ... 281 lines not shown
```

instrain_amd/csrc/obs_encode.h:

```cpp
#pragma once
#include <stdint.h>

#include <condition_variable>
#include <functional>
#include <mutex>
#include <thread>
#include <vector>

#include "../../include/instrain_amd.h"

namespace isxenc {

class HostPool {
public:
    HostPool(int n_threads, int numa_node, bool pin);
    ~HostPool();
    int size() const { return (int)th_.size() + 1; }
    void run(int n_tasks, const std::function<void(int)> &fn);

private:
    void worker(int idx);
    std::vector<std::thread> th_;
    std::vector<std::vector<int>> cpus_;
    std::mutex mu_;
    std::condition_variable cv_, cv_done_;
    const std::function<void(int)> *fn_ = nullptr;
    int n_tasks_ = 0, next_ = 0, running_ = 0;
    uint64_t gen_ = 0;
    bool stop_ = false;
};

struct PairRun { uint32_t first, pair; };

struct EncodeJob {
    const isx_obs *obs = nullptr;
    const uint32_t *pair = nullptr;
    std::function<void(int64_t first, uint32_t count, isx_obs *obs_out, uint32_t *pair_out)> produce;
    bool want_pairs = false;
    int64_t n_obs = 0, n_pos = 0;
    int record_bytes = 2;
    void *rec = nullptr;
    uint32_t *gbase = nullptr;
    uint32_t *pair_out = nullptr;
    PairRun *runs_out = nullptr;
    size_t cap_runs = 0;
    uint32_t *run_index_out = nullptr;
    size_t n_runs = 0;
    uint32_t *cmin = nullptr, *cmax = nullptr;
    uint8_t *cany = nullptr;
    int64_t cap_rec = 0;
    int64_t ring_groups = 0;
    std::function<void(int half)> wave_begin;
    std::function<void(int half, int64_t g0, int64_t g1)> wave_flush;
    double slack = 0.0;
    int64_t n_rec = 0;
    int64_t n_groups_real = 0;
    int64_t n_groups_in = 0;
    uint32_t max_pair = 0;
    int passes = 0;
};

enum { ENC_OK = 0, ENC_CAPACITY = 1, ENC_MM_RANGE = 2, ENC_BAD_POS = 3 };

int encode_obs(HostPool &pool, EncodeJob &job);

const char *encode_isa();

}
```

instrain_amd/csrc/seg_encode.cpp:

```cpp
#include "seg_encode.h"

#include <immintrin.h>

#include <algorithm>
#include <atomic>
#include <cstdlib>
#include <cstring>
#include <string>
#include <vector>

void isx_set_error(const std::string &msg);

namespace isxenc {

namespace {

constexpr int64_t TASK = 4096;
constexpr uint32_t SPAN = 65535u;

inline int64_t count_groups(const uint32_t *gpos, int64_t a, int64_t e, int64_t group = ISX_SEG_GROUP)
{
    int64_t n = 0;
    for (int64_t i = a; i < e;) {
        uint32_t lo = gpos[i], hi = gpos[i];
// ... 532 lines not shown
#define ISX_PLANES_PREFETCH 16
#endif
constexpr int64_t PLANES_PREFETCH = ISX_PLANES_PREFETCH;
struct PlaneGroup {
    alignas(64) uint32_t rec[ISX_DREC_GROUP][ISX_DREC_WORDS];
    int n = 0, open = -1;
    uint32_t lo = 0, hi = 0, last = 0;
    int64_t g = 0, used = 0;
};
__attribute__((noinline)) void rebase_drecs(PlaneGroup &G, uint32_t new_lo)
{
    const uint32_t up = G.lo - new_lo;
    for (int r = 0; r < G.n; r++) {
        uint32_t *o = G.rec[r];
        if ((o[0] >> 16) & 0xFFu) o[0] += up;
        if ((o[0] & ISX_DREC_DUAL) && ((o[4] >> 16) & 0xFFu)) o[4] += up;
    }
    G.lo = new_lo;
}

struct PlaneScratch {
    std::vector<uint32_t> gpos, pair;
    std::vector<uint8_t> len, mm;
    std::vector<uint64_t> planes;
    uint64_t *pl = nullptr;
};

#define ISX_PLANES_FN planes_task_portable
#define ISX_CLOSE_FN close_group_portable
#define ISX_DIFFERS_FN differs160_portable
#define ISX_PLANES_VARIANT 0
#include "seg_planes.inc"
#undef ISX_PLANES_FN
#undef ISX_CLOSE_FN
#undef ISX_DIFFERS_FN
#undef ISX_PLANES_VARIANT
#pragma GCC push_options
#pragma GCC target("bmi,bmi2,popcnt,lzcnt")
#define ISX_PLANES_FN planes_task_bmi2
#define ISX_CLOSE_FN close_group_bmi2
#define ISX_DIFFERS_FN differs160_bmi2
#define ISX_PLANES_VARIANT 1
#include "seg_planes.inc"
#undef ISX_PLANES_FN
#undef ISX_CLOSE_FN
#undef ISX_DIFFERS_FN
#undef ISX_PLANES_VARIANT
#pragma GCC pop_options
#pragma GCC push_options
#pragma GCC target("bmi,bmi2,popcnt,lzcnt,avx512f,avx512bw,avx512vl,avx512vbmi2,gfni")
#define ISX_PLANES_FN planes_task_avx512
#define ISX_CLOSE_FN close_group_avx512
#define ISX_DIFFERS_FN differs160_avx512
#define ISX_PLANES_VARIANT 2
#include "seg_planes.inc"
#undef ISX_PLANES_FN
#undef ISX_CLOSE_FN
#undef ISX_DIFFERS_FN
#undef ISX_PLANES_VARIANT
#pragma GCC pop_options

inline int planes_variant()
{
    static const int v = [] {
        if (const char *e = getenv("ISX_PLANES_VARIANT")) return std::max(0, std::min(2, atoi(e)));
        if (!cpu_has_bmi2()) return 0;
        return cpu_has_avx512() && __builtin_cpu_supports("avx512vbmi2") && __builtin_cpu_supports("gfni") ? 2 : 1;
    }();
    if (v == 2 && !(cpu_has_avx512() && __builtin_cpu_supports("avx512vbmi2") && __builtin_cpu_supports("gfni") && __builtin_cpu_supports("bmi2"))) return __builtin_cpu_supports("bmi2") ? 1 : 0;
    if (v == 1 && !__builtin_cpu_supports("bmi2")) return 0;
    return v;
}

}

int encode_planes(HostPool &pool, SegJob &J)
{
    const int64_t n = J.n_seg;
    const bool producer = (bool)J.produce_planes;
    const uint32_t *gpos_all = producer ? J.gpos_all : J.in2.gpos;
    const int n_tasks = (int)((n + TASK - 1) / TASK);
    const int64_t slack = std::max<int64_t>(J.slack_groups, 1);
    std::vector<int64_t> g_at((size_t)n_tasks + 1, 0);
    if (J.task_groups) for (int t = 0; t < n_tasks; t++) g_at[(size_t)t + 1] = std::max<int64_t>(J.task_groups[t], 1);
    else pool.run(n_tasks, [&](int t) {
        const int64_t a = (int64_t)t * TASK, e = std::min<int64_t>(n, a + TASK);
        g_at[(size_t)t + 1] = count_groups(gpos_all, a, e, 2 * ISX_DREC_GROUP) + slack;
    });
    for (int t = 0; t < n_tasks; t++) g_at[(size_t)t + 1] += g_at[(size_t)t];
    const int64_t n_groups = std::max<int64_t>(g_at[(size_t)n_tasks], 1);
    J.n_rec = n_groups * ISX_DREC_GROUP;
    J.need_slack = slack;
    if (J.n_rec > J.cap_rec) return SEG_CAPACITY;
    std::atomic<int> err{SEG_OK};
    std::vector<int64_t> bases_of((size_t)std::max(n_tasks, 1), 0), need_of((size_t)std::max(n_tasks, 1), 0), pieces_of((size_t)std::max(n_tasks, 1), 0);
    std::vector<uint32_t> maxp_of((size_t)std::max(n_tasks, 1), 0);
    const bool pairs = producer ? J.want_pairs : J.in2.pair != nullptr;
    const int64_t RG = J.ring_groups;
    constexpr size_t group_words = (size_t)ISX_DREC_GROUP * ISX_DREC_WORDS;
    const bool fast_store = cpu_has_avx512() && (reinterpret_cast<uintptr_t>(J.rec) & 63) == 0;
    const int variant = planes_variant();
    if (n == 0) {
        if (RG) J.wave_begin(0);
        for (int r = 0; r < ISX_DREC_GROUP; r++) put_empty_drec(J.rec + (size_t)r * ISX_DREC_WORDS);
        J.gbase[0] = 0; J.cmin[0] = 0xFFFFFFFFu; J.cmax[0] = 0; J.cany[0] = 0;
        J.n_bases = 0; J.max_pair = 0; J.n_pieces = 0;
        if (RG) J.wave_flush(0, 0, 1);
        return SEG_OK;
    }
    auto run_task = [&](int t, int64_t wave_g0, int half) {
        if (err.load(std::memory_order_relaxed) != SEG_OK) return;
        const int64_t a = (int64_t)t * TASK, e = std::min<int64_t>(n, a + TASK);
        const uint32_t *gp, *pr;
        const uint8_t *ln, *mmv = nullptr;
        const uint64_t *pl;
        if (producer) {
            thread_local PlaneScratch S;
            if (S.gpos.size() < (size_t)TASK) {
                S.gpos.resize((size_t)TASK); S.pair.resize((size_t)TASK); S.len.resize((size_t)TASK); S.mm.resize((size_t)TASK);
                S.planes.resize((size_t)TASK * ISX_PLANE_WORDS + 8);
                S.pl = reinterpret_cast<uint64_t *>((reinterpret_cast<uintptr_t>(S.planes.data()) + 63) & ~(uintptr_t)63);
            }
            J.produce_planes(a, e - a, S.gpos.data(), S.len.data(), J.n_mm_bins > 1 ? S.mm.data() : nullptr, pairs ? S.pair.data() : nullptr, S.pl);
            gp = S.gpos.data() - a; ln = S.len.data() - a; pr = pairs ? S.pair.data() - a : nullptr;
            if (J.n_mm_bins > 1) mmv = S.mm.data() - a;
            pl = S.pl - (size_t)a * ISX_PLANE_WORDS;
        } else {
            gp = J.in2.gpos; ln = J.in2.len; pr = pairs ? J.in2.pair : nullptr; pl = J.in2.planes;
            if (J.n_mm_bins > 1) mmv = J.in2.mm;
        }
        PlaneTask K;
        K.a = a; K.e = e; K.gp = gp; K.ln = ln; K.mm = mmv; K.pr = pr; K.pl = pl; K.gpos_all = gpos_all;
        K.rec0 = RG ? J.rec + (size_t)((int64_t)half * RG) * group_words : J.rec;
        K.g0 = RG ? wave_g0 : 0; K.ga = g_at[(size_t)t]; K.ge = g_at[(size_t)t + 1]; K.fast_store = fast_store;
        if (variant == 2) planes_task_avx512(J, err, K);
        else if (variant == 1) planes_task_bmi2(J, err, K);
        else planes_task_portable(J, err, K);
        if (err.load(std::memory_order_relaxed) != SEG_OK) return;
        need_of[(size_t)t] = K.used;
        bases_of[(size_t)t] = K.nb; maxp_of[(size_t)t] = K.maxp; pieces_of[(size_t)t] = K.np;
    };
    if (!RG) pool.run(n_tasks, [&](int t) { run_task(t, 0, 0); });
    else {
        int half = 0;
        for (int t0 = 0; t0 < n_tasks && err.load() == SEG_OK;) {
            int t1 = t0 + 1;
            while (t1 < n_tasks && g_at[(size_t)t1 + 1] - g_at[(size_t)t0] <= RG) t1++;
            if (g_at[(size_t)t1] - g_at[(size_t)t0] > RG) return SEG_CAPACITY;
            J.wave_begin(half);
            const int64_t wg0 = g_at[(size_t)t0];
            pool.run(t1 - t0, [&](int k) { run_task(t0 + k, wg0, half); });
            if (err.load() == SEG_OK) J.wave_flush(half, wg0, g_at[(size_t)t1]);
            t0 = t1; half ^= 1;
        }
    }
    if (err.load() != SEG_OK) return err.load();
    J.n_bases = 0; J.max_pair = 0; J.n_pieces = 0;
    int64_t worst = 0;
    bool fits = true;
    J.task_need.assign(need_of.begin(), need_of.begin() + n_tasks);
    for (int t = 0; t < n_tasks; t++) {
        J.n_bases += bases_of[(size_t)t]; J.max_pair = std::max(J.max_pair, maxp_of[(size_t)t]); J.n_pieces += pieces_of[(size_t)t];
        const int64_t region = g_at[(size_t)t + 1] - g_at[(size_t)t];
        if (need_of[(size_t)t] > region) fits = false;
        worst = std::max(worst, need_of[(size_t)t] - (region - (J.task_groups ? 0 : slack)));
    }
    J.need_slack = fits ? slack : std::max<int64_t>(worst, slack + 1);
    if (!fits) return SEG_CAPACITY;
    return SEG_OK;
}


namespace {
__attribute__((target("bmi2")))
inline void pack_ref_piece_bmi2(const uint8_t *r, int64_t n, uint8_t *o2, uint8_t *on, bool &seen)
{
    int64_t i = 0;
    uint64_t any = 0;
    for (; i + 8 <= n; i += 8) {
        uint64_t x;
        memcpy(&x, r + i, 8);
        const uint64_t bad = x & 0xFCFCFCFCFCFCFCFCull;
        if (__builtin_expect(bad == 0, 1)) {
            const uint16_t v = (uint16_t)_pext_u64(x, 0x0303030303030303ull);
            memcpy(o2 + (i >> 2), &v, 2);
            on[i >> 3] = 0;
            continue;
        }
        uint64_t t = bad | (bad >> 4);
        t |= t >> 2; t |= t >> 1;
        const uint64_t nb = t & 0x0101010101010101ull;
        const uint64_t keep = ~(nb * 0xFFull);
        const uint16_t v = (uint16_t)_pext_u64(x & keep, 0x0303030303030303ull);
        memcpy(o2 + (i >> 2), &v, 2);
        on[i >> 3] = (uint8_t)_pext_u64(nb, 0x0101010101010101ull);
        any |= nb;
    }
    for (; i < n; i += 8) {
        uint32_t lo = 0, hi = 0, nbits = 0;
        const int64_t m = std::min<int64_t>(8, n - i);
        for (int64_t k = 0; k < m; k++) {
            const uint32_t c = r[i + k];
            const uint32_t b = c > 3u;
            nbits |= b << k;
            const uint32_t v = b ? 0u : c;
            if (k < 4) lo |= v << (2 * k); else hi |= v << (2 * (k - 4));
        }
        o2[i >> 2] = (uint8_t)lo;
        if (m > 4) o2[(i >> 2) + 1] = (uint8_t)hi;
        on[i >> 3] = (uint8_t)nbits;
        any |= nbits;
    }
    seen = any != 0;
}

inline void pack_ref_piece_scalar(const uint8_t *r, int64_t n, uint8_t *o2, uint8_t *on, bool &seen)
{
    seen = false;
    for (int64_t i = 0; i < n; i += 8) {
        uint32_t lo = 0, hi = 0, nb = 0;
        const int64_t m = std::min<int64_t>(8, n - i);
        for (int64_t k = 0; k < m; k++) {
            const uint32_t c = r[i + k];
            const uint32_t bad = c > 3u;
            nb |= bad << k;
            const uint32_t v = bad ? 0u : c;
            if (k < 4) lo |= v << (2 * k); else hi |= v << (2 * (k - 4));
        }
        o2[i >> 2] = (uint8_t)lo;
        if (m > 4) o2[(i >> 2) + 1] = (uint8_t)hi;
        on[i >> 3] = (uint8_t)nb;
        seen |= nb != 0;
    }
}
}

bool pack_ref_planes(HostPool &pool, const uint8_t *ref, int64_t n_pos, uint8_t *plane2, uint8_t *nplane)
{
    const int64_t piece = (int64_t)256 << 10;
    const int n_tasks = (int)((n_pos + piece - 1) / piece);
    std::atomic<int> any{0};
    const bool bmi2 = cpu_has_bmi2();
    auto cp = [&](int t) {
        const int64_t a = (int64_t)t * piece, e = std::min<int64_t>(n_pos, a + piece);
        bool seen = false;
        if (bmi2) pack_ref_piece_bmi2(ref + a, e - a, plane2 + (a >> 2), nplane + (a >> 3), seen);
        else pack_ref_piece_scalar(ref + a, e - a, plane2 + (a >> 2), nplane + (a >> 3), seen);
        if (seen) any.store(1, std::memory_order_relaxed);
    };
    if (n_tasks > 1) pool.run(n_tasks, cp); else if (n_tasks == 1) cp(0);
    return any.load() != 0;
}
// ... 207 lines not shown
    }
    if (bad) { isx_set_error("isx_pack_reads: a CIGAR reaches beyond its read's bases or the flat space"); return ISX_ERR_ARG; }
    if (full) { isx_set_error("isx_pack_reads: more segments than cap_seg (isx_count_read_segs gives the number)"); return ISX_ERR_CAPACITY; }
    *n_seg = n;
    return ISX_OK;
}

int isx_pack_ref_planes(const uint8_t *ref, int64_t n_pos, int32_t host_threads, uint8_t *plane2, uint8_t *nplane, int32_t *has_n)
{
    if (!ref || n_pos <= 0 || !plane2 || !nplane) { isx_set_error("isx_pack_ref_planes: bad argument"); return ISX_ERR_ARG; }
    isxenc::HostPool pool(std::max(1, host_threads), -1, false);
    const bool any = isxenc::pack_ref_planes(pool, ref, n_pos, plane2, nplane);
    if (has_n) *has_n = any ? 1 : 0;
    return ISX_OK;
}

int isx_planes_from_segs(const isx_segs *segs, int32_t host_threads, uint64_t *planes)
{
    if (!segs || segs->n_seg < 0 || (segs->n_seg && (!segs->len || !segs->bases || !planes))) { isx_set_error("isx_planes_from_segs: bad argument"); return ISX_ERR_ARG; }
    const int64_t n = segs->n_seg, piece = 8192;
    std::atomic<bool> bad{false};
    isxenc::HostPool pool(std::max(1, host_threads), -1, false);
    pool.run((int)((n + piece - 1) / piece), [&](int t) {
        const int64_t a = (int64_t)t * piece, e = std::min<int64_t>(n, a + piece);
        for (int64_t i = a; i < e; i++) {
            const uint32_t L = segs->len[i];
            if (L == 0 || L > ISX_SEG_BASES) { bad.store(true); return; }
            isxenc::planes_from_words(segs->bases + (size_t)i * ISX_SEG_WORDS, L, planes + (size_t)i * ISX_PLANE_WORDS);
        }
    });
    if (bad.load()) { isx_set_error("a segment's length is not in [1, 150]"); return ISX_ERR_ARG; }
    return ISX_OK;
}

int isx_encode_planes(const isx_read_planes *reads, const isx_ref_planes *ref, int64_t n_pos, int32_t host_threads, int32_t slack_groups,
                      int64_t cap_rec, int64_t ring_records, uint32_t *rec, uint32_t *gbase, int64_t *n_rec, int64_t *need_slack)
{
    return isx_encode_planes_mm(reads, ref, n_pos, 1, host_threads, slack_groups, cap_rec, ring_records, rec, gbase, n_rec, need_slack);
}

int isx_encode_planes_mm(const isx_read_planes *reads, const isx_ref_planes *ref, int64_t n_pos, int32_t n_mm_bins, int32_t host_threads, int32_t slack_groups,
                         int64_t cap_rec, int64_t ring_records, uint32_t *rec, uint32_t *gbase, int64_t *n_rec, int64_t *need_slack)
{
    if (n_mm_bins < 1 || n_mm_bins > 128) { isx_set_error("isx_encode_planes: n_mm_bins must be in [1, 128]"); return ISX_ERR_ARG; }
    if (!reads || !ref || !ref->plane2 || !rec || !gbase || !n_rec || reads->n_seg < 0 || cap_rec < ISX_DREC_GROUP || (cap_rec % ISX_DREC_GROUP) || n_pos <= 0 ||
        (reads->n_seg && (!reads->gpos || !reads->len || !reads->planes)) || ring_records < 0 ||
        (ring_records % (2 * ISX_DREC_GROUP)) || slack_groups < 0) {
        isx_set_error("isx_encode_planes: bad argument");
        return ISX_ERR_ARG;
    }
    std::vector<uint32_t> ring;
    isxenc::HostPool pool(std::max(1, host_threads), -1, false);
    std::vector<uint32_t> cmin((size_t)(cap_rec / ISX_DREC_GROUP)), cmax(cmin.size());
    std::vector<uint8_t> cany(cmin.size());
    isxenc::SegJob J;
    J.in2 = *reads; J.n_seg = reads->n_seg; J.n_pos = n_pos; J.n_mm_bins = n_mm_bins;
    J.ref2 = ref->plane2; J.refn = ref->nplane; J.slack_groups = std::max(1, slack_groups);
    J.rec = rec; J.gbase = gbase; J.pair_out = nullptr;
    J.cmin = cmin.data(); J.cmax = cmax.data(); J.cany = cany.data(); J.cap_rec = cap_rec;
    if (ring_records) {
        const int64_t half = ring_records / 2;
        ring.assign((size_t)ring_records * ISX_DREC_WORDS + 16, 0xABABABABu);
        uint32_t *r0 = reinterpret_cast<uint32_t *>((reinterpret_cast<uintptr_t>(ring.data()) + 63) & ~(uintptr_t)63);
        J.rec = r0;
        J.ring_groups = half / ISX_DREC_GROUP;
        J.wave_begin = [](int) {};
        J.wave_flush = [&, r0](int h, int64_t g0, int64_t g1) {
            const size_t gw = (size_t)ISX_DREC_GROUP * ISX_DREC_WORDS;
            memcpy(rec + (size_t)g0 * gw, r0 + (size_t)h * half * ISX_DREC_WORDS, (size_t)(g1 - g0) * gw * 4);
            std::fill_n(r0 + (size_t)h * half * ISX_DREC_WORDS, (size_t)half * ISX_DREC_WORDS, 0xABABABABu);
        };
    }
    const int rc = isxenc::encode_planes(pool, J);
    if (need_slack) *need_slack = J.need_slack;
    *n_rec = J.n_rec;
    if (rc == isxenc::SEG_CAPACITY) {
        isx_set_error(J.need_slack > J.slack_groups ? "isx_encode_planes: a task needs more spare groups than slack_groups (see *need_slack)"
                                                    : "isx_encode_planes: the stream does not fit cap_rec records");
        return ISX_ERR_CAPACITY;
    }
    if (rc == isxenc::SEG_BAD_POS) { isx_set_error("a segment reaches beyond n_pos"); return ISX_ERR_ARG; }
    if (rc == isxenc::SEG_BAD_LEN) { isx_set_error("a segment's length is not in [1, 150]"); return ISX_ERR_ARG; }
    if (rc == isxenc::SEG_MM_RANGE) { isx_set_error("a segment has mm >= n_mm_bins"); return ISX_ERR_MM_RANGE; }
    return ISX_OK;
}

int isx_pack_read_planes(int64_t n_reads, const int64_t *ref_start, const int64_t *clip_lo, const int64_t *clip_hi,
                         const uint32_t *cigar, const int64_t *cigar_off, const char *seq, const uint8_t *qual, const int64_t *seq_off,
                         const uint32_t *pair, int32_t min_base_quality, int64_t cap_seg, uint32_t *seg_gpos,
                         uint8_t *seg_len, uint32_t *seg_pair, uint64_t *seg_planes, int64_t *n_seg)
{
    if (n_reads < 0 || !n_seg || cap_seg < 0 || (n_reads && (!ref_start || !clip_lo || !clip_hi || !cigar || !cigar_off || !seq || !qual || !seq_off)) ||
        (cap_seg && (!seg_gpos || !seg_len || !seg_planes)) || (pair && cap_seg && !seg_pair)) {
        isx_set_error("isx_pack_read_planes: bad argument");
        return ISX_ERR_ARG;
    }
    int64_t n = 0;
    bool full = false, bad = false;
    for (int64_t r = 0; r < n_reads && !full && !bad; r++) {
        const char *sq = seq + seq_off[r];
        const uint8_t *ql = qual + seq_off[r];
        const int64_t q_len = seq_off[r + 1] - seq_off[r];
        const bool ok = for_runs(cigar + cigar_off[r], cigar_off[r + 1] - cigar_off[r], ref_start[r], clip_lo[r], clip_hi[r],
                                 [&](int64_t pos, int64_t q0, int64_t cols) {
            if (q0 + cols > q_len || pos < 0 || pos + cols > (int64_t)0xFFFFFFFFll) { bad = true; return; }
            for (int64_t c0 = 0; c0 < cols && !full; c0 += ISX_SEG_BASES) {
                const int L = (int)std::min<int64_t>(ISX_SEG_BASES, cols - c0);
                if (n >= cap_seg) { full = true; return; }
                uint64_t *P = seg_planes + (size_t)n * ISX_PLANE_WORDS;
                for (int k = 0; k < ISX_PLANE_WORDS; k++) P[k] = 0;
                for (int j = 0; j < L; j++) {
                    const int64_t qi = q0 + c0 + j;
                    const uint32_t code = (int)ql[qi] >= min_base_quality ? ascii_code(sq[qi]) : 4u;
                    if (code >= 4) {
                        P[5 + (j >> 6)] |= (uint64_t)1 << (j & 63);
                        if (code == 5) { P[j >> 5] |= (uint64_t)1 << (2 * (j & 31)); P[7] |= (uint64_t)1 << 63; }
                    } else P[j >> 5] |= (uint64_t)code << (2 * (j & 31));
                }
                seg_gpos[n] = (uint32_t)(pos + c0); seg_len[n] = (uint8_t)L;
                if (seg_pair) seg_pair[n] = pair ? pair[r] : 0u;
                n++;
            }
        });
        if (!ok) { isx_set_error("isx_pack_read_planes: unknown CIGAR operator"); return ISX_ERR_ARG; }
    }
    if (bad) { isx_set_error("isx_pack_read_planes: a CIGAR reaches beyond its read's bases or the flat space"); return ISX_ERR_ARG; }
    if (full) { isx_set_error("isx_pack_read_planes: more segments than cap_seg (isx_count_read_segs gives the number)"); return ISX_ERR_CAPACITY; }
    *n_seg = n;
    return ISX_OK;
}

}
```

instrain_amd/csrc/seg_encode.h:

```cpp
#pragma once
#include <stdint.h>

#include <functional>
#include <vector>

#include "../../include/instrain_amd.h"
#include "obs_encode.h"

#define ISX_SEG_GROUP 16
#define ISX_SEG_REC_WORDS 16
#define ISX_DREC_GROUP 32

namespace isxenc {

struct SegJob {
    isx_segs in{};
    std::function<void(int64_t first, int64_t count, uint32_t *gpos, uint8_t *len, uint8_t *mm, uint32_t *pair, uint32_t *bases)> produce;
    const uint32_t *gpos_all = nullptr;
    isx_read_planes in2{};
    std::function<void(int64_t first, int64_t count, uint32_t *gpos, uint8_t *len, uint8_t *mm, uint32_t *pair, uint64_t *planes)> produce_planes;
    const uint8_t *ref2 = nullptr, *refn = nullptr;
    int64_t n_seg = 0, n_pos = 0;
    int n_mm_bins = 1;
    bool want_pairs = false;
    uint32_t *rec = nullptr;
    uint32_t *gbase = nullptr;
    uint32_t *pair_out = nullptr;
    uint32_t *cmin = nullptr, *cmax = nullptr;
    uint8_t *cany = nullptr;
    int64_t cap_rec = 0;
    int64_t ring_groups = 0;
    std::function<void(int half)> wave_begin;
    std::function<void(int half, int64_t g0, int64_t g1)> wave_flush;
    const uint8_t *ref = nullptr;
    int64_t slack_groups = 1;
    int64_t need_slack = 0;
    std::vector<int64_t> task_need;
    const int64_t *task_groups = nullptr;
    int64_t n_pieces = 0;
    int64_t n_rec = 0;
    int64_t n_bases = 0;
    uint32_t max_pair = 0;
};

enum { SEG_OK = 0, SEG_CAPACITY = 1, SEG_MM_RANGE = 2, SEG_BAD_POS = 3, SEG_BAD_LEN = 4 };

int encode_segs(HostPool &pool, SegJob &job);
int encode_delta(HostPool &pool, SegJob &job);
int encode_planes(HostPool &pool, SegJob &job);
int64_t delta_groups_needed(HostPool &pool, const uint32_t *gpos, int64_t n, int64_t slack_groups);
int64_t seg_groups_needed(HostPool &pool, const uint32_t *gpos, int64_t n);
bool pack_ref_planes(HostPool &pool, const uint8_t *ref, int64_t n_pos, uint8_t *plane2, uint8_t *nplane);
void planes_from_words(const uint32_t *words, uint32_t len, uint64_t *planes);

}
```

instrain_amd/engine.py:

```python
import ctypes as C
import os

import numpy as np

from . import _lib
from ._lib import (ENTRY_DT, LD_DT, OBS_DT, SNV_DT, BamInfo, BamParams, IsxError, Params, Sizes,
                   Timings, check)


def pack_obs(gpos, base, mm):
    o = np.empty(len(gpos), dtype=OBS_DT)
    o["gpos"] = gpos
    o["mm"] = mm
    o["base"] = base
    o["flags"] = 0
    return o


class SegBatch:

    def __init__(self, gpos, length, bases, mm=None, pair=None):
        self.gpos = np.ascontiguousarray(gpos, dtype=np.uint32)
        self.len = np.ascontiguousarray(length, dtype=np.uint8)
        self.bases = np.ascontiguousarray(bases, dtype=np.uint32).reshape(-1, _lib.SEG_WORDS)
# ... 801 lines not shown
        pass


def encode_obs(obs, pair=None, n_pos=None, record_bytes=2, threads=1, slack=0.0, cap_rec=None, ring_records=0):
    lib = _lib.load()
    obs = np.ascontiguousarray(obs, dtype=OBS_DT)
    G = 512 if record_bytes == 2 else 256
    if cap_rec is None:
        cap_rec = (int(len(obs) * 1.5) + 4 * 2048 + 2047) // 2048 * 2048
    if n_pos is None:
        n_pos = int(obs["gpos"].max()) + 1 if len(obs) else 1
    rec = np.empty(cap_rec, dtype=np.uint16 if record_bytes == 2 else np.uint32)
    gbase = np.empty(cap_rec // G, dtype=np.uint32)
    pout = np.empty(cap_rec, dtype=np.uint32) if pair is not None else None
    if pair is not None:
        pair = np.ascontiguousarray(pair, dtype=np.uint32)
    n_rec, passes = C.c_int64(0), C.c_int32(0)
    check(lib.isx_encode_obs_ring(obs.ctypes.data if len(obs) else None, pair.ctypes.data if pair is not None else None, len(obs),
                                  int(n_pos), int(record_bytes), int(threads), float(slack), int(cap_rec), int(ring_records),
                                  rec.ctypes.data, gbase.ctypes.data, pout.ctypes.data if pout is not None else None,
                                  C.byref(n_rec), C.byref(passes)))
    n = n_rec.value
    return rec[:n], gbase[:n // G], (pout[:n] if pout is not None else None), passes.value


def dense_clon(cov, clon_sparse, min_cov):
    out = np.where(np.asarray(cov) >= min_cov, np.float32(1.0), np.float32(np.nan)).astype(np.float32)
    out[clon_sparse["gpos"]] = clon_sparse["clon"]
    return out


def encode_segs(segs, n_pos, n_mm_bins=1, threads=1, cap_rec=None, ring_records=0):
    lib = _lib.load()
    if cap_rec is None:
        cap_rec = int(lib.isx_seg_records_needed(segs.gpos.ctypes.data if segs.n_seg else None, segs.n_seg, int(threads)))
    rec = np.empty((cap_rec, 16), dtype=np.uint32)
    gbase = np.empty(cap_rec // 16, dtype=np.uint32)
    pout = np.empty(cap_rec, dtype=np.uint32) if segs.pair is not None else None
    n_rec = C.c_int64(0)
    cs = segs.c()
    check(lib.isx_encode_segs_ring(C.byref(cs), int(n_pos), int(n_mm_bins), int(threads), int(cap_rec), int(ring_records), rec.ctypes.data,
                                   gbase.ctypes.data, pout.ctypes.data if pout is not None else None, C.byref(n_rec)))
    n = n_rec.value
    return rec[:n], gbase[:n // 16], (pout[:n] if pout is not None else None)


def encode_delta(segs, ref_codes, n_mm_bins=1, threads=1, slack_groups=1, cap_rec=None, ring_records=0, retry=True):
    lib = _lib.load()
    ref = np.ascontiguousarray(ref_codes, dtype=np.uint8)
    while True:
        cap = cap_rec if cap_rec is not None else int(lib.isx_delta_records_needed(segs.gpos.ctypes.data if segs.n_seg else None, segs.n_seg, int(threads), int(slack_groups)))
        rec = np.empty((cap, 8), dtype=np.uint32)
        gbase = np.empty(cap // 32, dtype=np.uint32)
        n_rec, need = C.c_int64(0), C.c_int64(0)
        cs = segs.c()
        rc = lib.isx_encode_delta(C.byref(cs), ref.ctypes.data, len(ref), int(n_mm_bins), int(threads), int(slack_groups), cap, int(ring_records),
                                  rec.ctypes.data, gbase.ctypes.data, None, C.byref(n_rec), C.byref(need))
        if rc == _lib.ERR_CAPACITY and retry and need.value > slack_groups and cap_rec is None:
            slack_groups = int(need.value)
            continue
        check(rc)
        n = n_rec.value
        return rec[:n], gbase[:n // 32], None, slack_groups


def encode_planes(reads, ref_planes, threads=1, slack_groups=1, cap_rec=None, ring_records=0, retry=True, n_mm_bins=1):
    lib = _lib.load()
    while True:
        cap = cap_rec if cap_rec is not None else int(lib.isx_delta_records_needed(reads.gpos.ctypes.data if reads.n_seg else None, reads.n_seg, int(threads), int(slack_groups)))
        rec = _aligned((cap, 8), np.uint32)
        gbase = np.empty(cap // 32, dtype=np.uint32)
        n_rec, need = C.c_int64(0), C.c_int64(0)
        cr, cf = reads.c(), ref_planes.c()
        rc = lib.isx_encode_planes_mm(C.byref(cr), C.byref(cf), ref_planes.n_pos, int(n_mm_bins), int(threads), int(slack_groups), cap, int(ring_records),
                                      rec.ctypes.data, gbase.ctypes.data, C.byref(n_rec), C.byref(need))
        if rc == _lib.ERR_CAPACITY and retry and need.value > slack_groups and cap_rec is None:
            slack_groups = int(need.value)
            continue
        check(rc)
        n = n_rec.value
        return rec[:n], gbase[:n // 32], None, slack_groups


def dense_cov(res, n_pos=None):
    if "cov16" in res:
        return res["cov16"]
    if "cov8" in res:
        cov = res["cov8"].astype(np.uint16)
    else:
        nib = res["cov4"]
        n_pos = 2 * len(nib) if n_pos is None else int(n_pos)
        cov = np.empty(2 * len(nib), dtype=np.uint16)
        cov[0::2] = nib & 15
        cov[1::2] = nib >> 4
        cov = cov[:n_pos]
        W = int(res["cov_window"])
        for k, w in enumerate(res["cov_row_win"].tolist()):
            lo = w * W
            hi = min(lo + W, n_pos)
            cov[lo:hi] = res["cov_rows"][k, :hi - lo]
    if "saturated" in res:
        cov[res["saturated"]["gpos"]] = np.minimum(res["saturated"]["coverage"], 65535)
    return cov


DREC_DUAL = 0x80000000
DREC_NO_EXC = 0x3FFFFFFF


def decode_delta(rec, gbase, ref_codes):
    rec = np.asarray(rec, dtype=np.uint32).reshape(-1, 8)
    ref = np.asarray(ref_codes, dtype=np.uint8)
    n = len(rec)
    dual = (rec[:, 0] >> 31) == 1
    assert ((rec[dual, 4] >> 31) == 1).all(), "a dual record's second half carries the flag too"
    zero = np.zeros(n, dtype=np.uint32)
    none = np.full(n, DREC_NO_EXC, dtype=np.uint32)
    hdr = np.stack([rec[:, 0], np.where(dual, rec[:, 4], zero)], axis=1)
    pair = np.stack([np.where(dual, rec[:, 1], rec[:, 7]), np.where(dual, rec[:, 5], zero)], axis=1)
    e0 = np.stack([np.where(dual, rec[:, 2], rec[:, 3]), np.where(dual, rec[:, 6], none)], axis=1)
    e1 = np.stack([np.where(dual, rec[:, 3], none), np.where(dual, rec[:, 7], none)], axis=1)
    skw = [np.stack([np.where(dual, zero, rec[:, k]), zero], axis=1) for k in (1, 2, 4, 5, 6)]
    gb = np.repeat(np.asarray(gbase, dtype=np.uint32), 32)[:n]
    start = (gb[:, None] + (hdr & 0xFFFF)).astype(np.int64)
    ln = ((hdr >> 16) & 0xFF).astype(np.int64)
    lvl = ((hdr >> 24) & 0x7F).astype(np.uint8)
    full = np.stack([~dual, np.zeros(n, dtype=bool)], axis=1)
    real = (ln > 0).reshape(-1)
    flat = lambda x: x.reshape(-1)[real]
    st, ln, pr, e0, e1, fl, lvl = flat(start), flat(ln), flat(pair), flat(e0), flat(e1), flat(full), flat(lvl)
    words = np.stack([flat(w) for w in skw], axis=1)
    m = len(st)
    j = np.arange(160, dtype=np.int64)[None, :]
    skip = ((words[:, :, None] >> np.arange(32, dtype=np.uint32)[None, None, :]) & 1).reshape(m, 160).astype(bool)
    assert not (skip & (j >= ln[:, None])).any(), "skip bits beyond a piece's length"
    assert skip[fl].any(axis=1).all() or True
    inside = j < ln[:, None]
    pos = np.minimum(st[:, None] + j, len(ref) - 1)
    codes = np.where(inside & ~skip, ref[pos], 4).astype(np.uint8)
    for e in (e0, e1):
        for k in range(3):
            f = (e >> (10 * k)) & 0x3FF
            has = f != 0x3FF
            off, base = (f & 0xFF).astype(np.int64), ((f >> 8) & 3).astype(np.uint8)
            rows = np.flatnonzero(has)
            assert (off[rows] < ln[rows]).all()
            mark = skip[rows, off[rows]]
            assert fl[rows[mark]].all(), "a non-ACGT marker in a dual half"
            codes[rows[mark], off[rows[mark]]] = 5
            rows = rows[~mark]
            assert (base[rows] != ref[st[rows] + off[rows]]).all(), "an exception that equals the reference"
            codes[rows, off[rows]] = base[rows]
        assert ((e >> 30) == 0).all()
    return st.astype(np.uint32), ln.astype(np.uint8), lvl, codes[:, :150], pr, fl


def decode_segs(rec, gbase):
    rec = np.asarray(rec, dtype=np.uint32).reshape(-1, 16)
    hdr = rec[:, 0]
    ln = (hdr >> 16) & 0xFF
    real = ln > 0
    start = np.repeat(np.asarray(gbase, dtype=np.uint32), 16)[:len(rec)] + (hdr & 0xFFFF)
    return start[real], ln[real].astype(np.uint8), (hdr[real] >> 24).astype(np.uint8), unpack_codes(rec[real, 1:])


def pack_reads(ref_start, clip_lo, clip_hi, cigars, seqs, quals, mm=None, pair=None, min_base_quality=30):
# ... 316 lines not shown
```

Baseline: 170.7.

## Fuse window-directory build into the record pass's host thread pool phases

Reworks the host thread pool to run multi-phase jobs, with spin-then-sleep phase barriers instead of separate pool.run dispatches. The window-directory build (prefix max/suffix min, then per-window range search) becomes a two-phase DirJob. In the plane-input path it is appended as tail phases of the record encoding pass, so choose_windows can reuse the already built directory instead of building it again. This is meant to save the dispatch and wake-up latency of separate pool runs, at the cost of a more complex barrier and speculatively building the directory for the first window size tried.

```diff
diff --git a/include/instrain_amd.h b/include/instrain_amd.h
--- a/include/instrain_amd.h
+++ b/include/instrain_amd.h
@@ -499,6 +499,8 @@
                       int64_t cap_rec, int64_t ring_records, uint32_t *rec, uint32_t *gbase, int64_t *n_rec, int64_t *need_slack);
 int isx_encode_planes_mm(const isx_read_planes *reads, const isx_ref_planes *ref, int64_t n_pos, int32_t n_mm_bins, int32_t host_threads, int32_t slack_groups,
                          int64_t cap_rec, int64_t ring_records, uint32_t *rec, uint32_t *gbase, int64_t *n_rec, int64_t *need_slack);
+int isx_encode_planes_dir(const isx_read_planes *reads, const isx_ref_planes *ref, int64_t n_pos, int32_t host_threads, int32_t slack_groups, int32_t repeats,
+                          int64_t cap_rec, uint32_t *rec, uint32_t *gbase, int64_t *n_rec, int32_t window, uint32_t *win, int64_t *longest);
 
 int isx_count_read_segs(int64_t n_reads, const uint32_t *cigar, const int64_t *cigar_off, const int64_t *ref_start,
                         const int64_t *clip_lo, const int64_t *clip_hi, int64_t *n_seg);
diff --git a/instrain_amd/_lib.py b/instrain_amd/_lib.py
--- a/instrain_amd/_lib.py
+++ b/instrain_amd/_lib.py
@@ -179,7 +179,7 @@
            "isx_irep_layout", "isx_irep_create", "isx_irep_destroy", "isx_irep_sizes", "isx_irep_add", "isx_irep_blocks_fetch", "isx_irep_blocks_add", "isx_irep_finish",
            "isx_genes_create", "isx_genes_destroy", "isx_genes_sites", "isx_batch_profile_genes", "isx_genes_profile_snvs",
            "isx_pipe_create", "isx_pipe_destroy", "isx_pipe_submit", "isx_pipe_submit_reads", "isx_pipe_stage_reads", "isx_pipe_submit_wire", "isx_wire_bytes", "isx_wire_free", "isx_wire_keep_reference", "isx_pipe_submit_bam", "isx_encode_segs", "isx_encode_segs_ring", "isx_seg_records_needed", "isx_encode_delta", "isx_delta_records_needed", "isx_count_read_segs", "isx_pack_reads", "isx_pipe_collect", "isx_pipe_release", "isx_pipe_fetch_entries", "isx_pipe_fetch_entries_shrunk", "isx_levels_expand", "isx_encode_obs", "isx_encode_obs_ring",
-           "isx_pack_ref_planes", "isx_planes_from_segs", "isx_pack_read_planes", "isx_pipe_submit_planes", "isx_pipe_stage_planes", "isx_encode_planes", "isx_encode_planes_mm", "isx_pipe_set_reference_budget", "isx_host_register", "isx_host_unregister",
+           "isx_pack_ref_planes", "isx_planes_from_segs", "isx_pack_read_planes", "isx_pipe_submit_planes", "isx_pipe_stage_planes", "isx_encode_planes", "isx_encode_planes_mm", "isx_encode_planes_dir", "isx_pipe_set_reference_budget", "isx_host_register", "isx_host_unregister",
            "isx_bgzf_index", "isx_bgzf_inflate_device", "isx_bgzf_inflate_host", "isx_bgzf_inflate_fast",
            "isx_bam_open", "isx_bam_close", "isx_bam_close_wait", "isx_bam_set_threads", "isx_bam_ref", "isx_bam_set_priority_reads", "isx_bam_scan", "isx_bam_scan_part",
            "isx_bam_insert_sizes", "isx_bam_set_wanted_refs", "isx_bam_pair_keys", "isx_bam_set_cross_names", "isx_bam_filter_insert_sizes", "isx_bam_filter", "isx_bam_set_r2m", "isx_bam_r2m", "isx_bam_drop_names", "isx_bam_batch_pair_names", "isx_bam_set_mm_cap", "isx_bam_mm_levels", "isx_bam_set_mm_levels", "isx_bam_ref_counts",
@@ -332,6 +332,7 @@
     lib.isx_host_unregister.argtypes = [vp]
     lib.isx_pipe_stage_planes.argtypes = [vp, i64, C.POINTER(RefPlanes), i32, vp, C.POINTER(ReadPlanes), C.POINTER(vp)]
     lib.isx_encode_planes.argtypes = [C.POINTER(ReadPlanes), C.POINTER(RefPlanes), i64, i32, i32, i64, i64, vp, vp, C.POINTER(i64), C.POINTER(i64)]
+    lib.isx_encode_planes_dir.argtypes = [C.POINTER(ReadPlanes), C.POINTER(RefPlanes), i64, i32, i32, i32, i64, vp, vp, C.POINTER(i64), i32, vp, C.POINTER(i64)]
     lib.isx_encode_planes_mm.argtypes = [C.POINTER(ReadPlanes), C.POINTER(RefPlanes), i64, i32, i32, i32, i64, i64, vp, vp, C.POINTER(i64), C.POINTER(i64)]
     lib.isx_bam_ref.argtypes = [vp, i32, C.POINTER(C.c_char_p), C.POINTER(i64), C.POINTER(i64)]
     lib.isx_bam_copy.argtypes = [vp, vp, vp, vp, vp]
diff --git a/instrain_amd/csrc/isx_api.hip b/instrain_amd/csrc/isx_api.hip
--- a/instrain_amd/csrc/isx_api.hip
+++ b/instrain_amd/csrc/isx_api.hip
@@ -767,70 +767,50 @@
     return longest;
 }
 
+static void check_directory(const uint32_t *cmin, const uint32_t *cmax, const uint8_t *cany, uint64_t n_chunks, int W, int64_t n_pos,
+                            const std::vector<uint2> &win, uint32_t chunk, uint64_t longest, const char *who)
+{
+    std::vector<uint2> ref;
+    const uint64_t l2 = build_window_directory(cmin, cmax, cany, n_chunks, W, n_pos, ref, chunk);
+    if (l2 != longest || ref.size() != win.size() || memcmp(ref.data(), win.data(), ref.size() * sizeof(uint2)) != 0) {
+        fprintf(stderr, "%s differs from build_window_directory (%llu chunks, %llu windows)\n", who, (unsigned long long)n_chunks, (unsigned long long)ref.size());
+        abort();
+    }
+}
+
 static uint64_t build_window_directory_mt(isxenc::HostPool &pool, const uint32_t *cmin, const uint32_t *cmax, const uint8_t *cany, uint64_t n_chunks, int W,
                                           int64_t n_pos, std::vector<uint2> &win, uint32_t chunk, std::vector<uint32_t> &pmax, std::vector<uint32_t> &smin)
 {
     const int n_win = (int)((n_pos + W - 1) / W);
     const int T = std::min(pool.size(), 16);
-    if (T < 2 || n_chunks < 4096 || n_win < 1024) return build_window_directory(cmin, cmax, cany, n_chunks, W, n_pos, win, chunk);
-    if (pmax.size() < n_chunks) { pmax.resize(n_chunks); smin.resize(n_chunks); }
-    const uint64_t B = (n_chunks + (uint64_t)T - 1) / (uint64_t)T;
-    uint32_t bmax[16], bmin[16], cmax_in[16], cmin_in[16];
-    pool.run(T, [&](int t) {
-        const uint64_t a = std::min(n_chunks, B * (uint64_t)t), e = std::min(n_chunks, a + B);
-        uint32_t run = 0;
-        for (uint64_t i = a; i < e; i++) { if (cany[i]) run = std::max(run, cmax[i]); pmax[i] = run; }
-        bmax[t] = run;
-        run = 0xFFFFFFFFu;
-        for (uint64_t i = e; i-- > a;) { if (cany[i]) run = std::min(run, cmin[i]); smin[i] = run; }
-        bmin[t] = run;
-    });
-    { uint32_t run = 0; for (int t = 0; t < T; t++) { cmax_in[t] = run; run = std::max(run, bmax[t]); } }
-    { uint32_t run = 0xFFFFFFFFu; for (int t = T; t-- > 0;) { cmin_in[t] = run; run = std::min(run, bmin[t]); } }
-    auto PM = [&](uint64_t i) { return std::max(pmax[i], cmax_in[i / B]); };
-    auto SM = [&](uint64_t i) { return std::min(smin[i], cmin_in[i / B]); };
+    if (!directory_threads_pay(pool.size(), n_chunks, n_win)) return build_window_directory(cmin, cmax, cany, n_chunks, W, n_pos, win, chunk);
+    static_assert(sizeof(isxenc::WinRange) == sizeof(uint2), "a window's record range is a uint2");
     win.resize((size_t)n_win);
-    uint64_t longest_t[16];
-    pool.run(T, [&](int t) {
-        const int wa = (int)((int64_t)n_win * t / T), we = (int)((int64_t)n_win * (t + 1) / T);
-        uint64_t longest = 0, lo = 0, hi = 0;
-        if (wa < we) {
-            const uint64_t w0 = (uint64_t)wa * (uint64_t)W;
-            uint64_t l = 0, r = n_chunks;
-            while (l < r) { const uint64_t m = (l + r) >> 1; if ((uint64_t)PM(m) < w0) l = m + 1; else r = m; }
-            lo = hi = l;
-        }
-        for (int w = wa; w < we; w++) {
-            const uint64_t w0 = (uint64_t)w * (uint64_t)W, w1 = w0 + (uint64_t)W;
-            while (lo < n_chunks && (uint64_t)PM(lo) < w0) lo++;
-            if (hi < lo) hi = lo;
-            while (hi < n_chunks && (uint64_t)SM(hi) < w1) hi++;
-            win[(size_t)w] = make_uint2((uint32_t)(lo * chunk), (uint32_t)(hi * chunk));
-            longest = std::max(longest, (hi - lo) * chunk);
-        }
-        longest_t[t] = longest;
-    });
-    uint64_t longest = 0;
-    for (int t = 0; t < T; t++) longest = std::max(longest, longest_t[t]);
-    if (getenv("ISX_DIR_CHECK")) {
-        std::vector<uint2> ref;
-        const uint64_t l2 = build_window_directory(cmin, cmax, cany, n_chunks, W, n_pos, ref, chunk);
-        if (l2 != longest || ref.size() != win.size() || memcmp(ref.data(), win.data(), ref.size() * sizeof(uint2)) != 0) {
-            fprintf(stderr, "build_window_directory_mt differs from build_window_directory (%llu chunks, %d windows)\n", (unsigned long long)n_chunks, n_win);
-            abort();
-        }
-    }
+    isxenc::DirJob D;
+    D.cmin = cmin; D.cmax = cmax; D.cany = cany; D.n_chunks = n_chunks; D.chunk = chunk; D.W = W; D.n_pos = n_pos; D.T = T;
+    D.pmax = &pmax; D.smin = &smin; D.win = reinterpret_cast<isxenc::WinRange *>(win.data());
+    pool.run_phases(isxenc::DirJob::PHASES, [&](int ph) { return D.count(ph); }, [&](int ph, int t) { D.task(ph, t); });
+    const uint64_t longest = D.longest();
+    if (getenv("ISX_DIR_CHECK")) check_directory(cmin, cmax, cany, n_chunks, W, n_pos, win, chunk, longest, "build_window_directory_mt");
     return longest;
 }
 
-int choose_windows(const isx_batch *b, int64_t n_pos, const ChunkDir &dir, DirThreads *mt, std::vector<uint2> &win, int *packed)
-{
-    auto build = [&](int W) {
+static bool packed_counters_allowed(const isx_batch *b) { return (b->M > 1 || b->drec) && !(b->prm.layout & ISX_LAYOUT_NO_PACKED_COUNTERS); }
+
+int first_window_tried(const isx_batch *b, int64_t n_pos) { return batch_window_for(b, n_pos, packed_counters_allowed(b)); }
+
+int choose_windows(const isx_batch *b, int64_t n_pos, const ChunkDir &dir, DirThreads *mt, std::vector<uint2> &win, int *packed, const DirBuilt *built)
+{
+    auto build = [&](int W) -> uint64_t {
+        if (built && built->W == W && win.size() == (size_t)((n_pos + W - 1) / W)) {
+            if (getenv("ISX_DIR_CHECK")) check_directory(dir.cmin, dir.cmax, dir.cany, dir.n_chunks, W, n_pos, win, dir.chunk, built->longest, "the record pass' window directory");
+            return built->longest;
+        }
         return mt ? build_window_directory_mt(mt->pool, dir.cmin, dir.cmax, dir.cany, dir.n_chunks, W, n_pos, win, dir.chunk, mt->pmax, mt->smin)
                   : build_window_directory(dir.cmin, dir.cmax, dir.cany, dir.n_chunks, W, n_pos, win, dir.chunk);
     };
     *packed = 0;
-    if ((b->M > 1 || b->drec) && !(b->prm.layout & ISX_LAYOUT_NO_PACKED_COUNTERS)) {
+    if (packed_counters_allowed(b)) {
         const int Wp = batch_window_for(b, n_pos, true);
         if (build(Wp) < (b->drec ? 32768u : 65536u)) { *packed = 1; return Wp; }
     }
diff --git a/instrain_amd/csrc/isx_batch.h b/instrain_amd/csrc/isx_batch.h
--- a/instrain_amd/csrc/isx_batch.h
+++ b/instrain_amd/csrc/isx_batch.h
@@ -138,7 +138,11 @@
 
 struct ChunkDir { const uint32_t *cmin, *cmax; const uint8_t *cany; uint64_t n_chunks; uint32_t chunk; };
 struct DirThreads { isxenc::HostPool &pool; std::vector<uint32_t> &pmax, &smin; };
-int choose_windows(const isx_batch *b, int64_t n_pos, const ChunkDir &dir, DirThreads *mt, std::vector<uint2> &win, int *packed);
+struct DirBuilt { int W; uint64_t longest; };
+int choose_windows(const isx_batch *b, int64_t n_pos, const ChunkDir &dir, DirThreads *mt, std::vector<uint2> &win, int *packed, const DirBuilt *built = nullptr);
+inline bool directory_threads_pay(int pool_size, uint64_t n_chunks, int64_t n_win) { return pool_size >= 2 && n_chunks >= 4096 && n_win >= 1024; }
+inline bool fused_directory_pays(int pool_size, int64_t n_seg, int64_t n_pos, int W) { return directory_threads_pay(pool_size, (uint64_t)n_seg / 64, (n_pos + W - 1) / W); }
+int first_window_tried(const isx_batch *b, int64_t n_pos);
 
 int batch_set_geometry(isx_batch *b);
 
diff --git a/instrain_amd/csrc/isx_pipe.hip b/instrain_amd/csrc/isx_pipe.hip
--- a/instrain_amd/csrc/isx_pipe.hip
+++ b/instrain_amd/csrc/isx_pipe.hip
@@ -51,6 +51,7 @@
     size_t in_bytes = 0;
     size_t off_bounds = 0, off_win = 0, off_ref = 0, off_gbase = 0, off_ridx = 0, off_rec = 0;
     size_t off_pairs = 0;
+    isxenc::DirJob dir_job;
     isxenc::PairRun *h_runs = nullptr;
     bool runs_pinned = true;
     uint2 *d_runs = nullptr;
@@ -1018,12 +1019,12 @@
     return ISX_OK;
 }
 
-static int slot_choose_windows(isx_pipe *p, Slot &s, uint32_t chunk, bool threads)
+static int slot_choose_windows(isx_pipe *p, Slot &s, uint32_t chunk, bool threads, const DirBuilt *built = nullptr)
 {
     isx_batch *b = s.b;
     DirThreads mt{*p->pool, s.dir_pmax, s.dir_smin};
     const ChunkDir dir{s.cmin.data(), s.cmax.data(), s.cany.data(), b->n_rec / chunk, chunk};
-    b->W = choose_windows(b, b->n_pos, dir, threads ? &mt : nullptr, s.win, &b->packed);
+    b->W = choose_windows(b, b->n_pos, dir, threads ? &mt : nullptr, s.win, &b->packed, built);
     b->n_win = (int)s.win.size();
     if (s.win.size() > (size_t)p->pp.max_pos / 64 + 2) { isx_set_error("internal: window directory larger than the arena"); return ISX_ERR_STATE; }
     memcpy(s.h_in + s.off_win, s.win.data(), s.win.size() * sizeof(uint2));
@@ -1304,6 +1305,18 @@
         if ((rc = stage_reference(p, s, n_pos, ref, rp, J, &rs)) != ISX_OK) return rc;
     }
     if (p->drec) J.ref = ref;
+    isxenc::DirJob &D = s.dir_job;
+    if (planes_in && !ring && fused_directory_pays(p->pool->size(), J.n_seg, n_pos, first_window_tried(b, n_pos))) {
+        D = isxenc::DirJob();
+        D.cmin = s.cmin.data(); D.cmax = s.cmax.data(); D.cany = s.cany.data(); D.chunk = p->G;
+        D.W = first_window_tried(b, n_pos); D.n_pos = n_pos; D.T = std::min(p->pool->size(), 16);
+        D.pmax = &s.dir_pmax; D.smin = &s.dir_smin;
+        s.win.resize((size_t)((n_pos + D.W - 1) / D.W));
+        D.win = reinterpret_cast<isxenc::WinRange *>(s.win.data());
+        J.tail_phases = isxenc::DirJob::PHASES;
+        J.tail_count = [&D, &J, p](int ph) { if (ph == 0) D.n_chunks = (uint64_t)(J.n_rec / (int64_t)p->G); return D.count(ph); };
+        J.tail_fn = [&D](int ph, int t) { D.task(ph, t); };
+    }
     const int erc = encode_reads(p, s, J, planes_in, feed);
     const double t_enc = now_ms();
     if (feed.err != hipSuccess) { isx_set_error(std::string("isx_pipe_submit_reads: staging ring: ") + hipGetErrorString(feed.err)); return ISX_ERR_HIP; }
@@ -1327,7 +1340,8 @@
 
     b->n_pos = n_pos; b->n_obs = J.n_bases; b->n_splits = n_splits; b->n_rec = (uint64_t)J.n_rec;
     b->n_pairs = (uint64_t)J.max_pair + 1;
-    if ((rc = slot_choose_windows(p, s, p->G, true)) != ISX_OK) return rc;
+    const DirBuilt built{D.W, J.tail_ran ? D.longest() : 0};
+    if ((rc = slot_choose_windows(p, s, p->G, true, J.tail_ran ? &built : nullptr)) != ISX_OK) return rc;
     if ((rc = slot_shape_pass(p, s)) != ISX_OK) return rc;
     slot_bind_inputs(p, s, rs.resident);
     s.encode_ms = (float)(now_ms() - t0);
diff --git a/instrain_amd/csrc/obs_encode.cpp b/instrain_amd/csrc/obs_encode.cpp
--- a/instrain_amd/csrc/obs_encode.cpp
+++ b/instrain_amd/csrc/obs_encode.cpp
@@ -5,6 +5,7 @@
 
 #include <algorithm>
 #include <atomic>
+#include <chrono>
 #include <cstdio>
 #include <cstring>
 #include <map>
@@ -109,36 +110,74 @@
         cv_.wait(lk, [&] { return stop_ || gen_ != seen; });
         if (stop_) return;
         seen = gen_;
-        while (next_ < n_tasks_) {
-            const int t = next_++;
-            const auto *fn = fn_;
-            lk.unlock();
-            (*fn)(t);
-            lk.lock();
-        }
+        lk.unlock();
+        work_phases();
+        lk.lock();
         if (--running_ == 0) cv_done_.notify_all();
     }
 }
 
-void HostPool::run(int n_tasks, const std::function<void(int)> &fn)
-{
-    if (n_tasks <= 0) return;
+void HostPool::work_phases()
+{
+    const int n_threads = (int)th_.size() + 1;
+    const auto &fn = *fn_;
+    for (int ph = 0;; ph++) {
+        const int n = ph_tasks_;
+        for (;;) {
+            if (next_.load(std::memory_order_relaxed) >= n) break;
+            const int t = next_.fetch_add(1, std::memory_order_relaxed);
+            if (t >= n) break;
+            fn(ph, t);
+        }
+        if (ph + 1 == n_phases_) return;
+        if (arrived_.fetch_add(1, std::memory_order_acq_rel) + 1 == n_threads) {
+            ph_tasks_ = std::max(0, (*count_)(ph + 1));
+            next_.store(0, std::memory_order_relaxed);
+            arrived_.store(0, std::memory_order_relaxed);
+            phase_.store(ph + 1, std::memory_order_release);
+            std::lock_guard<std::mutex> lk(mu_);
+            if (sleepers_) cv_phase_.notify_all();
+            continue;
+        }
+        bool open = false;
+        const auto t0 = std::chrono::steady_clock::now();
+        for (int spin = 0; !(open = phase_.load(std::memory_order_acquire) > ph); spin++) {
+            __builtin_ia32_pause();
+            if ((spin & 63) == 63 && std::chrono::steady_clock::now() - t0 > std::chrono::microseconds(50)) break;
+        }
+        if (!open) {
+            std::unique_lock<std::mutex> lk(mu_);
+            sleepers_++;
+            cv_phase_.wait(lk, [&] { return phase_.load(std::memory_order_acquire) > ph; });
+            sleepers_--;
+        }
+    }
+}
+
+void HostPool::run_phases(int n_phases, const std::function<int(int)> &count, const std::function<void(int, int)> &fn)
+{
+    if (n_phases <= 0) return;
+    const int n0 = std::max(0, count(0));
+    if (n_phases == 1 && n0 == 0) return;
     std::unique_lock<std::mutex> lk(mu_);
-    fn_ = &fn; n_tasks_ = n_tasks; next_ = 0;
+    fn_ = &fn; count_ = &count; n_phases_ = n_phases;
+    ph_tasks_ = n0;
+    next_.store(0, std::memory_order_relaxed); arrived_.store(0, std::memory_order_relaxed); phase_.store(0, std::memory_order_relaxed);
     running_ = (int)th_.size() + 1;
     ++gen_;
     lk.unlock();
     cv_.notify_all();
+    work_phases();
     lk.lock();
-    while (next_ < n_tasks_) {
-        const int t = next_++;
-        lk.unlock();
-        fn(t);
-        lk.lock();
-    }
     --running_;
     cv_done_.wait(lk, [&] { return running_ == 0; });
-    fn_ = nullptr;
+    fn_ = nullptr; count_ = nullptr;
+}
+
+void HostPool::run(int n_tasks, const std::function<void(int)> &fn)
+{
+    if (n_tasks <= 0) return;
+    run_phases(1, [n_tasks](int) { return n_tasks; }, [&fn](int, int t) { fn(t); });
 }
 
 namespace {
diff --git a/instrain_amd/csrc/obs_encode.h b/instrain_amd/csrc/obs_encode.h
--- a/instrain_amd/csrc/obs_encode.h
+++ b/instrain_amd/csrc/obs_encode.h
@@ -1,6 +1,7 @@
 #pragma once
 #include <stdint.h>
 
+#include <atomic>
 #include <condition_variable>
 #include <functional>
 #include <mutex>
@@ -17,15 +18,24 @@
     ~HostPool();
     int size() const { return (int)th_.size() + 1; }
     void run(int n_tasks, const std::function<void(int)> &fn);
+    void run_phases(int n_phases, const std::function<int(int)> &count, const std::function<void(int, int)> &fn);
 
 private:
     void worker(int idx);
+    void work_phases();
     std::vector<std::thread> th_;
     std::vector<std::vector<int>> cpus_;
     std::mutex mu_;
     std::condition_variable cv_, cv_done_;
-    const std::function<void(int)> *fn_ = nullptr;
-    int n_tasks_ = 0, next_ = 0, running_ = 0;
+    const std::function<void(int, int)> *fn_ = nullptr;
+    const std::function<int(int)> *count_ = nullptr;
+    int n_phases_ = 0, running_ = 0;
+    int ph_tasks_ = 0;
+    alignas(64) std::atomic<int> next_{0};
+    alignas(64) std::atomic<int> arrived_{0};
+    alignas(64) std::atomic<int> phase_{0};
+    int sleepers_ = 0;
+    std::condition_variable cv_phase_;
     uint64_t gen_ = 0;
     bool stop_ = false;
 };
diff --git a/instrain_amd/csrc/seg_encode.cpp b/instrain_amd/csrc/seg_encode.cpp
--- a/instrain_amd/csrc/seg_encode.cpp
+++ b/instrain_amd/csrc/seg_encode.cpp
@@ -638,21 +638,27 @@
     const int n_tasks = (int)((n + TASK - 1) / TASK);
     const int64_t slack = std::max<int64_t>(J.slack_groups, 1);
     std::vector<int64_t> g_at((size_t)n_tasks + 1, 0);
-    if (J.task_groups) for (int t = 0; t < n_tasks; t++) g_at[(size_t)t + 1] = std::max<int64_t>(J.task_groups[t], 1);
-    else pool.run(n_tasks, [&](int t) {
+    auto count_task = [&](int t) {
         const int64_t a = (int64_t)t * TASK, e = std::min<int64_t>(n, a + TASK);
         g_at[(size_t)t + 1] = count_groups(gpos_all, a, e, 2 * ISX_DREC_GROUP) + slack;
-    });
-    for (int t = 0; t < n_tasks; t++) g_at[(size_t)t + 1] += g_at[(size_t)t];
-    const int64_t n_groups = std::max<int64_t>(g_at[(size_t)n_tasks], 1);
-    J.n_rec = n_groups * ISX_DREC_GROUP;
-    J.need_slack = slack;
-    if (J.n_rec > J.cap_rec) return SEG_CAPACITY;
+    };
+    auto layout = [&]() -> bool {
+        if (J.task_groups) for (int t = 0; t < n_tasks; t++) g_at[(size_t)t + 1] = std::max<int64_t>(J.task_groups[t], 1);
+        for (int t = 0; t < n_tasks; t++) g_at[(size_t)t + 1] += g_at[(size_t)t];
+        J.n_rec = std::max<int64_t>(g_at[(size_t)n_tasks], 1) * ISX_DREC_GROUP;
+        J.need_slack = slack;
+        return J.n_rec <= J.cap_rec;
+    };
+    J.tail_ran = false;
+    const int64_t RG = J.ring_groups;
+    if (RG || n == 0) {
+        if (!J.task_groups) pool.run(n_tasks, count_task);
+        if (!layout()) return SEG_CAPACITY;
+    }
     std::atomic<int> err{SEG_OK};
     std::vector<int64_t> bases_of((size_t)std::max(n_tasks, 1), 0), need_of((size_t)std::max(n_tasks, 1), 0), pieces_of((size_t)std::max(n_tasks, 1), 0);
     std::vector<uint32_t> maxp_of((size_t)std::max(n_tasks, 1), 0);
     const bool pairs = producer ? J.want_pairs : J.in2.pair != nullptr;
-    const int64_t RG = J.ring_groups;
     constexpr size_t group_words = (size_t)ISX_DREC_GROUP * ISX_DREC_WORDS;
     const bool fast_store = cpu_has_avx512() && (reinterpret_cast<uintptr_t>(J.rec) & 63) == 0;
     const int variant = planes_variant();
@@ -696,34 +702,54 @@
         need_of[(size_t)t] = K.used;
         bases_of[(size_t)t] = K.nb; maxp_of[(size_t)t] = K.maxp; pieces_of[(size_t)t] = K.np;
     };
-    if (!RG) pool.run(n_tasks, [&](int t) { run_task(t, 0, 0); });
-    else {
-        int half = 0;
-        for (int t0 = 0; t0 < n_tasks && err.load() == SEG_OK;) {
-            int t1 = t0 + 1;
-            while (t1 < n_tasks && g_at[(size_t)t1 + 1] - g_at[(size_t)t0] <= RG) t1++;
-            if (g_at[(size_t)t1] - g_at[(size_t)t0] > RG) return SEG_CAPACITY;
-            J.wave_begin(half);
-            const int64_t wg0 = g_at[(size_t)t0];
-            pool.run(t1 - t0, [&](int k) { run_task(t0 + k, wg0, half); });
-            if (err.load() == SEG_OK) J.wave_flush(half, wg0, g_at[(size_t)t1]);
-            t0 = t1; half ^= 1;
-        }
-    }
-    if (err.load() != SEG_OK) return err.load();
-    J.n_bases = 0; J.max_pair = 0; J.n_pieces = 0;
-    int64_t worst = 0;
-    bool fits = true;
-    J.task_need.assign(need_of.begin(), need_of.begin() + n_tasks);
-    for (int t = 0; t < n_tasks; t++) {
-        J.n_bases += bases_of[(size_t)t]; J.max_pair = std::max(J.max_pair, maxp_of[(size_t)t]); J.n_pieces += pieces_of[(size_t)t];
-        const int64_t region = g_at[(size_t)t + 1] - g_at[(size_t)t];
-        if (need_of[(size_t)t] > region) fits = false;
-        worst = std::max(worst, need_of[(size_t)t] - (region - (J.task_groups ? 0 : slack)));
-    }
-    J.need_slack = fits ? slack : std::max<int64_t>(worst, slack + 1);
-    if (!fits) return SEG_CAPACITY;
-    return SEG_OK;
+    auto finish = [&]() -> int {
+        if (err.load() != SEG_OK) return err.load();
+        J.n_bases = 0; J.max_pair = 0; J.n_pieces = 0;
+        int64_t worst = 0;
+        bool fits = true;
+        J.task_need.assign(need_of.begin(), need_of.begin() + n_tasks);
+        for (int t = 0; t < n_tasks; t++) {
+            J.n_bases += bases_of[(size_t)t]; J.max_pair = std::max(J.max_pair, maxp_of[(size_t)t]); J.n_pieces += pieces_of[(size_t)t];
+            const int64_t region = g_at[(size_t)t + 1] - g_at[(size_t)t];
+            if (need_of[(size_t)t] > region) fits = false;
+            worst = std::max(worst, need_of[(size_t)t] - (region - (J.task_groups ? 0 : slack)));
+        }
+        J.need_slack = fits ? slack : std::max<int64_t>(worst, slack + 1);
+        return fits ? SEG_OK : SEG_CAPACITY;
+    };
+    if (!RG) {
+        bool fits_cap = false;
+        int status = -1;
+        const int tail = J.tail_fn && J.tail_count ? std::max(J.tail_phases, 0) : 0;
+        pool.run_phases(3 + tail,
+            [&](int ph) -> int {
+                if (ph == 0) return J.task_groups ? 0 : n_tasks;
+                if (ph == 1) return 1;
+                if (ph == 2) return fits_cap ? n_tasks : 0;
+                if (ph == 3) { status = fits_cap ? finish() : SEG_CAPACITY; J.tail_ran = status == SEG_OK; }
+                return J.tail_ran ? J.tail_count(ph - 3) : 0;
+            },
+            [&](int ph, int t) {
+                if (ph == 0) count_task(t);
+                else if (ph == 1) fits_cap = layout();
+                else if (ph == 2) run_task(t, 0, 0);
+                else J.tail_fn(ph - 3, t);
+            });
+        if (!fits_cap) return SEG_CAPACITY;
+        return status >= 0 ? status : finish();
+    }
+    int half = 0;
+    for (int t0 = 0; t0 < n_tasks && err.load() == SEG_OK;) {
+        int t1 = t0 + 1;
+        while (t1 < n_tasks && g_at[(size_t)t1 + 1] - g_at[(size_t)t0] <= RG) t1++;
+        if (g_at[(size_t)t1] - g_at[(size_t)t0] > RG) return SEG_CAPACITY;
+        J.wave_begin(half);
+        const int64_t wg0 = g_at[(size_t)t0];
+        pool.run(t1 - t0, [&](int k) { run_task(t0 + k, wg0, half); });
+        if (err.load() == SEG_OK) J.wave_flush(half, wg0, g_at[(size_t)t1]);
+        t0 = t1; half ^= 1;
+    }
+    return finish();
 }
 
 
@@ -1097,6 +1123,48 @@
     if (rc == isxenc::SEG_BAD_POS) { isx_set_error("a segment reaches beyond n_pos"); return ISX_ERR_ARG; }
     if (rc == isxenc::SEG_BAD_LEN) { isx_set_error("a segment's length is not in [1, 150]"); return ISX_ERR_ARG; }
     if (rc == isxenc::SEG_MM_RANGE) { isx_set_error("a segment has mm >= n_mm_bins"); return ISX_ERR_MM_RANGE; }
+    return ISX_OK;
+}
+
+int isx_encode_planes_dir(const isx_read_planes *reads, const isx_ref_planes *ref, int64_t n_pos, int32_t host_threads, int32_t slack_groups, int32_t repeats,
+                          int64_t cap_rec, uint32_t *rec, uint32_t *gbase, int64_t *n_rec, int32_t window, uint32_t *win, int64_t *longest)
+{
+    if (!reads || !ref || !ref->plane2 || !rec || !gbase || !n_rec || reads->n_seg < 0 || cap_rec < ISX_DREC_GROUP || (cap_rec % ISX_DREC_GROUP) || n_pos <= 0 ||
+        (reads->n_seg && (!reads->gpos || !reads->len || !reads->planes)) || slack_groups < 0 || repeats < 1 || window <= 0 || !win || !longest) {
+        isx_set_error("isx_encode_planes_dir: bad argument");
+        return ISX_ERR_ARG;
+    }
+    isxenc::HostPool pool(std::max(1, host_threads), -1, false);
+    std::vector<uint32_t> cmin((size_t)(cap_rec / ISX_DREC_GROUP)), cmax(cmin.size()), pmax, smin;
+    std::vector<uint8_t> cany(cmin.size());
+    isxenc::DirJob D;
+    int rc = isxenc::SEG_OK;
+    for (int32_t k = 0; k < repeats; k++) {
+        isxenc::SegJob J;
+        J.in2 = *reads; J.n_seg = reads->n_seg; J.n_pos = n_pos; J.n_mm_bins = 1;
+        J.ref2 = ref->plane2; J.refn = ref->nplane; J.slack_groups = std::max(1, slack_groups);
+        J.rec = rec; J.gbase = gbase; J.pair_out = nullptr;
+        J.cmin = cmin.data(); J.cmax = cmax.data(); J.cany = cany.data(); J.cap_rec = cap_rec;
+        D = isxenc::DirJob();
+        D.cmin = cmin.data(); D.cmax = cmax.data(); D.cany = cany.data(); D.chunk = ISX_DREC_GROUP;
+        D.W = window; D.n_pos = n_pos; D.T = std::min(pool.size(), 16);
+        D.pmax = &pmax; D.smin = &smin; D.win = reinterpret_cast<isxenc::WinRange *>(win);
+        J.tail_phases = isxenc::DirJob::PHASES;
+        J.tail_count = [&D, &J](int ph) { if (ph == 0) D.n_chunks = (uint64_t)(J.n_rec / ISX_DREC_GROUP); return D.count(ph); };
+        J.tail_fn = [&D](int ph, int t) { D.task(ph, t); };
+        rc = isxenc::encode_planes(pool, J);
+        *n_rec = J.n_rec;
+        if (rc != isxenc::SEG_OK) break;
+        if (!J.tail_ran) {
+            D.n_chunks = (uint64_t)(J.n_rec / ISX_DREC_GROUP);
+            pool.run_phases(isxenc::DirJob::PHASES, [&](int ph) { return D.count(ph); }, [&](int ph, int t) { D.task(ph, t); });
+        }
+        *longest = (int64_t)D.longest();
+    }
+    if (rc == isxenc::SEG_CAPACITY) { isx_set_error("isx_encode_planes_dir: the stream does not fit cap_rec records / slack_groups"); return ISX_ERR_CAPACITY; }
+    if (rc == isxenc::SEG_BAD_POS) { isx_set_error("a segment reaches beyond n_pos"); return ISX_ERR_ARG; }
+    if (rc == isxenc::SEG_BAD_LEN) { isx_set_error("a segment's length is not in [1, 150]"); return ISX_ERR_ARG; }
+    if (rc != isxenc::SEG_OK) { isx_set_error("isx_encode_planes_dir: the record pass failed"); return ISX_ERR_ARG; }
     return ISX_OK;
 }
 
diff --git a/instrain_amd/csrc/seg_encode.h b/instrain_amd/csrc/seg_encode.h
--- a/instrain_amd/csrc/seg_encode.h
+++ b/instrain_amd/csrc/seg_encode.h
@@ -1,6 +1,7 @@
 #pragma once
 #include <stdint.h>
 
+#include <algorithm>
 #include <functional>
 #include <vector>
 
@@ -38,9 +39,80 @@
     std::vector<int64_t> task_need;
     const int64_t *task_groups = nullptr;
     int64_t n_pieces = 0;
+    int tail_phases = 0;
+    std::function<int(int)> tail_count;
+    std::function<void(int, int)> tail_fn;
+    bool tail_ran = false;
     int64_t n_rec = 0;
     int64_t n_bases = 0;
     uint32_t max_pair = 0;
+};
+
+struct WinRange { uint32_t lo, hi; };
+struct DirJob {
+    const uint32_t *cmin = nullptr, *cmax = nullptr;
+    const uint8_t *cany = nullptr;
+    uint64_t n_chunks = 0;
+    uint32_t chunk = 1;
+    int W = 64;
+    int64_t n_pos = 0;
+    int T = 1;
+    std::vector<uint32_t> *pmax = nullptr, *smin = nullptr;
+    WinRange *win = nullptr;
+    uint64_t B = 1;
+    int n_win = 0;
+    uint32_t bmax[16], bmin[16], cmax_in[16], cmin_in[16];
+    uint64_t longest_t[16];
+    enum { PHASES = 2 };
+
+    int count(int ph)
+    {
+        if (ph == 0) {
+            T = std::max(1, std::min(T, 16));
+            n_win = (int)((n_pos + W - 1) / W);
+            if (pmax->size() < n_chunks) { pmax->resize(n_chunks); smin->resize(n_chunks); }
+            B = std::max<uint64_t>(1, (n_chunks + (uint64_t)T - 1) / (uint64_t)T);
+            return T;
+        }
+        { uint32_t run = 0; for (int t = 0; t < T; t++) { cmax_in[t] = run; run = std::max(run, bmax[t]); } }
+        { uint32_t run = 0xFFFFFFFFu; for (int t = T; t-- > 0;) { cmin_in[t] = run; run = std::min(run, bmin[t]); } }
+        return T;
+    }
+    void task(int ph, int t)
+    {
+        uint32_t *const pm = pmax->data(), *const sm = smin->data();
+        if (ph == 0) {
+            const uint64_t a = std::min(n_chunks, B * (uint64_t)t), e = std::min(n_chunks, a + B);
+            uint32_t run = 0;
+            for (uint64_t i = a; i < e; i++) { if (cany[i]) run = std::max(run, cmax[i]); pm[i] = run; }
+            bmax[t] = run;
+            run = 0xFFFFFFFFu;
+            for (uint64_t i = e; i-- > a;) { if (cany[i]) run = std::min(run, cmin[i]); sm[i] = run; }
+            bmin[t] = run;
+            return;
+        }
+        auto PM = [&](uint64_t i) { return std::max(pm[i], cmax_in[i / B]); };
+        auto SM = [&](uint64_t i) { return std::min(sm[i], cmin_in[i / B]); };
+        WinRange *const wn = win;
+        const int wa = (int)((int64_t)n_win * t / T), we = (int)((int64_t)n_win * (t + 1) / T);
+        uint64_t longest = 0, lo = 0, hi = 0;
+        if (wa < we) {
+            const uint64_t w0 = (uint64_t)wa * (uint64_t)W;
+            uint64_t l = 0, r = n_chunks;
+            while (l < r) { const uint64_t m = (l + r) >> 1; if ((uint64_t)PM(m) < w0) l = m + 1; else r = m; }
+            lo = hi = l;
+        }
+        for (int w = wa; w < we; w++) {
+            const uint64_t w0 = (uint64_t)w * (uint64_t)W, w1 = w0 + (uint64_t)W;
+            while (lo < n_chunks && (uint64_t)PM(lo) < w0) lo++;
+            if (hi < lo) hi = lo;
+            while (hi < n_chunks && (uint64_t)SM(hi) < w1) hi++;
+            wn[w].lo = (uint32_t)(lo * chunk); wn[w].hi = (uint32_t)(hi * chunk);
+            longest = std::max(longest, (hi - lo) * chunk);
+        }
+        longest_t[t] = longest;
+    }
+    uint64_t longest() const { uint64_t l = 0; for (int t = 0; t < T; t++) l = std::max(l, longest_t[t]); return l; }
 };
 
 enum { SEG_OK = 0, SEG_CAPACITY = 1, SEG_MM_RANGE = 2, SEG_BAD_POS = 3, SEG_BAD_LEN = 4 };
diff --git a/instrain_amd/engine.py b/instrain_amd/engine.py
--- a/instrain_amd/engine.py
+++ b/instrain_amd/engine.py
@@ -907,6 +907,21 @@
         return rec[:n], gbase[:n // 32], None, slack_groups
 
 
+def encode_planes_dir(reads, ref_planes, window, threads=1, slack_groups=1, repeats=1):
+    lib = _lib.load()
+    cap = int(lib.isx_delta_records_needed(reads.gpos.ctypes.data if reads.n_seg else None, reads.n_seg, int(threads), int(slack_groups)))
+    rec = _aligned((cap, 8), np.uint32)
+    gbase = np.empty(cap // 32, dtype=np.uint32)
+    n_win = (ref_planes.n_pos + window - 1) // window
+    win = np.zeros((n_win, 2), dtype=np.uint32)
+    n_rec, longest = C.c_int64(0), C.c_int64(0)
+    cr, cf = reads.c(), ref_planes.c()
+    check(lib.isx_encode_planes_dir(C.byref(cr), C.byref(cf), ref_planes.n_pos, int(threads), int(slack_groups), int(repeats), cap, rec.ctypes.data,
+                                    gbase.ctypes.data, C.byref(n_rec), int(window), win.ctypes.data, C.byref(longest)))
+    n = n_rec.value
+    return dict(rec=rec[:n], gbase=gbase[:n // 32], win=win, longest=longest.value)
+
+
 def dense_cov(res, n_pos=None):
     if "cov16" in res:
         return res["cov16"]
```

After: 169.8. No clear change (-0.5%).
